# facebookresearch/omni3d

Measured on AMD Instinct MI355X. Metric: images/sec train DLA34_FPN b=4/GPU, higher is better.
Workload: dtype f32; 1 GPU; cubercnn_DLA34_FPN train step, batch 4/GPU, synthetic Omni3D 512x512 (8 GT/img), fwd+10 losses+bwd+allreduce+divergence guard+SGD, random-init weights; global_batch=4, image=512x512, parallelism=dp1 (flat-bucket RCCL all-reduce)

## Files before the change

include/omni3d_hip.h:

```cpp
#ifndef OMNI3D_HIP_H
#define OMNI3D_HIP_H

#ifdef __cplusplus
extern "C" {
#endif


int omni_iou_box3d(const float* boxes1, int N, const float* boxes2, int M, const int* valid1, float* vol,
                   float* iou, int* overflow, void* stream);

int omni_iou_box3d_pairs(const float* boxes1, const float* boxes2, const int* idx1, const int* idx2,
                         long long npairs, const int* valid1, float* vol, float* iou, int* overflow,
                         void* stream);

int omni_iou_box3d_pairs_algo(const float* boxes1, const float* boxes2, const int* idx1, const int* idx2,
                              long long npairs, const int* valid1, float* vol, float* iou, int* overflow,
                              int lanes_per_pair, void* stream);

int omni_box3d_validity(const float* boxes, int N, float eps_coplanar, float eps_nonzero, int* valid,
                        int* counts, void* stream);


int omni_conv2d_fwd(const float* x, const float* w, const float* bias, float* out, int N, int H, int W, int C,
                    int K, int R, int S, int stride, int pad, int ldx, int ldo, int relu, void* stream);
// ... 160 lines not shown
int omni_rpn_collect(const float* boxes, const float* top_v, const int* top_i, int B, int N, int P, float* prop,
                     int* count, void* stream);

int omni_roi_sample(const float* prop_boxes, const int* prop_count, int B, int pmax, const float* gt,
                    const int* gt_cls, const int* gt_off, const float* ign, const int* ign_off, const float* expo,
                    float iou_thr, float ignore_thresh, float eps, int num_classes, int batch_per_image,
                    int nfg_max, int append_gt, float* out_boxes, int* out_cls, int* out_gt, float* out_iou,
                    int* out_counts, void* stream);
int omni_rpn_match_draw(const float* anchors, int A, const float* gt, const int* gt_off, int B, int G, float thr_lo,
                        float thr_hi, int l0, int l1, int l2, int allow_low_quality, const float* expo, long long* draw_state,
                        int* ticket, float eps, float* matched_val, int* matched_idx, signed char* match_label, int* gt_best_bits,
                        int* gt_best_idx, float* key_pos, float* key_neg, void* stream);
int omni_roi_sample_draw(const float* prop_boxes, const int* prop_count, int B, int pmax, const float* gt, const int* gt_cls,
                         const int* gt_off, const float* ign, const int* ign_off, const float* expo, long long* draw_state, int* ticket,
                         float iou_thr, float ignore_thresh, float eps, int num_classes, int batch_per_image, int nfg_max,
                         int append_gt, float* out_boxes, int* out_cls, int* out_gt, float* out_iou, int* out_counts, int* out_row,
                         int first, float* first_boxes, int* first_cls, int* first_row, void* stream);


int omni_roi_levels(const float* rois, int R, int min_level, int max_level, float canonical_size,
                    int canonical_level, int* levels, void* stream);

int omni_roi_align_fwd(const void* const* level_ptrs, const int* level_hw, const float* level_scale, int nlev,
                       const float* rois, const int* batch_idx, const int* levels, int R, int P, int C,
                       float* out, void* stream);
int omni_roi_align_fwd_mode(const void* const* level_ptrs, const int* level_hw, const float* level_scale, int nlev,
                            const float* rois, const int* batch_idx, const int* levels, int R, int P, int C, int aligned, float* out,
                            void* stream);
int omni_roi_align_bwd_mode(const void* const* dlevel_ptrs, const int* level_hw, const float* level_scale, int nlev,
                            const float* rois, const int* batch_idx, const int* levels, int R, int P, int C, int aligned,
                            const float* dout, void* stream);
int omni_roi_pool_fwd(const void* const* level_ptrs, const int* level_hw, const float* level_scale, int nlev, const float* rois,
                      const int* batch_idx, const int* levels, int R, int P, int C, float* out, int* argmax, void* stream);
int omni_roi_pool_bwd(const void* const* dlevel_ptrs, const int* level_hw, const float* level_scale, int nlev, const int* batch_idx,
                      const int* levels, int R, int P, int C, const float* dout, const int* argmax, void* stream);
int omni_roi_align_fwd2(const void* const* level_ptrs, const int* level_hw, const float* level_scale, int nlev,
                        const float* rois, const int* batch_idx, const int* levels, int R, int P, int C, float* out,
                        float* out2, int per_image, int first, void* stream);
int omni_roi_align_bwd(const void* const* dlevel_ptrs, const int* level_hw, const float* level_scale, int nlev,
                       const float* rois, const int* batch_idx, const int* levels, int R, int P, int C,
                       const float* dout, void* stream);
int omni_roi_align_bwd2(const void* const* dlevel_ptrs, const int* level_hw, const float* level_scale, int nlev,
                        const float* rois, const int* batch_idx, const int* levels, int R, int P, int C,
                        const float* dout, const float* dout2, int per_image, int first, void* stream);
int omni_roi_align_bwd_det(const void* const* dlevel_ptrs, const int* level_hw, const float* level_scale, int nlev, int B,
                           const float* rois, const int* batch_idx, const int* levels, int R, int P, int C, const float* dout,
                           const float* dout2, int per_image, int first, float* ws, long long ws_floats, int* ctr, int n_ctr,
                           long long* plan, void* stream);


int omni_box_loss_fwd(const float* pred, int ldp, int R, int K, const int* cls, const float* prop, const float* gt,
                      const int* gt_row, float wx, float wy, float ww, float wh, double* sums, void* stream);
int omni_box_loss_bwd(const float* pred, int ldp, int R, int K, const int* cls, const float* prop, const float* gt,
                      const int* gt_row, float wx, float wy, float ww, float wh, const double* sums,
                      const float* g_cls, const float* g_reg, float* dpred, void* stream);

int omni_box_decode_gt_class(const float* pred, int ldp, int R, int K, const int* cls, const float* prop, float wx, float wy,
                             float ww, float wh, float scale_clamp, float* out, void* stream);

int omni_cube_loss_fwd(const float* head, int ldh, int F, int K, int mode, int bins, const float* zscales, const float* zstats,
                       const float* boxes, const int* cls, const int* img,
                       const float* Ks, const float* v2r, const float* priors, const float* gt3d,
                       const float* gtpose, const int* gt_row, float w_dims, float w_pose, float w_xy, float w_z, float w_joint,
                       float* vals, float* jac, float* red, void* stream);
int omni_cube_loss_bwd(const float* vals, const float* jac, const float* red, const float* gk, const int* cls,
                       const float* boxes, int F, int K, int mode, int bins, const float* zscales, int ldh, float* dhead,
                       void* stream);
int omni_cube_decode(const float* head, int ldh, int F, int K, int mode, int bins, const float* zscales, const float* zstats,
                     const float* boxes, const int* cls, const int* img,
                     const float* Ks, const float* v2r, const float* ratio, const float* priors, float* cube3d,
                     float* pose, float* verts, void* stream);
int omni_cuboid_corners(const float* box3d, const float* R, int n, float* verts, void* stream);

int omni_conv2d_fwd_stats(const float* x, const float* w, float* out, int N, int H, int W, int C, int K, int R, int S,
                          int stride, int pad, int ldx, int ldo, float* stats, int stats_rows, int* nblk_out, void* stream);
int omni_wino_out_stats(const float* M, float* y, int N, int H, int W, int K, int tile, float* stats, int stats_rows,
                        int* nblk_out, void* stream);
int omni_wino_out_bn_bwd_stats(const float* M, float* y, int N, int H, int W, int K, int tile, const float* bn_x,
                               const float* mean_rstd, const float* scale_shift, float* stats, int stats_rows, int* nblk_out,
                               void* stream);
int omni_bn_bwd_partials(const float* x, const float* dy, const float* y, const float* gamma, const float* mean_rstd,
                         const float* partial, int nblk, float* dx, float* dres, float* dgamma, float* dbeta, float* coef,
                         int P, int C, int relu, int accumulate_param_grads, void* stream);
int omni_stem_conv_fwd_stats(const float* x, const float* w, float* out, int N, int H, int W, int C, int K, int R, int ldx,
                             int ldo, float* stats, int stats_rows, int* nblk_out, void* stream);
int omni_bn_fwd_partials(const float* x, const float* partial, int nblk, const float* gamma, const float* beta,
                         const float* residual, float* y, float* running_mean, float* running_var, float* mean_rstd,
                         float* scale_shift, int P, int C, float eps, float momentum, int relu, void* stream);

int omni_gemm_engine(const float* A, const float* B, float* C, const float* bias, int form, int batch, int M, int N, int K,
                     int lda, int ldb, int ldc, long long stride_a, long long stride_b, long long stride_c, int splits,
                     int relu, int accumulate, int tile, int workgroups, void* stream);
int omni_gemm_engine_det(const float* A, const float* B, float* C, const float* bias, int form, int batch, int M, int N, int K,
                         int lda, int ldb, int ldc, long long stride_a, long long stride_b, long long stride_c, int splits,
                         int relu, int accumulate, int tile, int workgroups, float* ws, long long ws_floats, int* ctr, int n_ctr,
                         long long* plan, void* stream);

int omni_transpose2d(const float* src, float* dst, int rows, int cols, void* stream);

int omni_det_scores(const float* pred, int ld, const float* rois, const int* count, const int* image_hw, int B, int P, int K,
                    float wx, float wy, float ww, float wh, float score_thresh, float* scores, float* probs, float* boxes,
                    void* stream);
int omni_det_nms_boxes(const float* boxes, const float* vals, const int* idx, int B, int PK, int K, int cap, float* nms_boxes,
                       int* valid, void* stream);
int omni_det_compact(const int* keep, const int* valid, const float* vals, const int* idx, const float* boxes, int B, int PK,
                     int K, int cap, int topk, float* out_box, float* out_score, int* out_cls, int* out_roi, int* out_count,
                     void* stream);

int omni_resize_bilinear_u8(const unsigned char* src, unsigned char* dst, unsigned char* tmp, int planes, int H, int W,
                            int HO, int WO, const int* bounds_h, const int* kk_h, int ksize_h, const int* bounds_v,
                            const int* kk_v, int ksize_v, int flip, void* stream);


int omni_sgd_step(float* param, const float* grad, float* momentum_buf, long long n, float lr, float momentum,
                  float dampening, float weight_decay, int nesterov, int first_step, float grad_scale,
                  const float* skip_flag, void* stream);
int omni_adam_step(float* param, const float* grad, float* exp_avg, float* exp_avg_sq, float* max_exp_avg_sq, long long n, float lr,
                   float beta1, float beta2, float eps, float weight_decay, int decoupled, const float* step, float grad_scale,
                   const float* skip_flag, void* stream);
int omni_adam_tick(float* step, const float* skip_flag, void* stream);
int omni_clip_norm_partials(const float* grad, const long long* tiles, int ntiles, float norm_type, double* partial, void* stream);
int omni_clip_norm_coef(const double* partial, const long long* ptab, int nparams, float norm_type, float max_norm, float grad_scale,
                        float* norm, float* coef, void* stream);
int omni_sgd_step_clipped(float* param, const float* grad, float* momentum_buf, const long long* tiles, int t0, int t1, int clip_mode,
                          const float* coef, float clip_value, float lr, float momentum, float dampening, float weight_decay,
                          int nesterov, int first_step, float grad_scale, const float* skip_flag, void* stream);
int omni_adam_step_clipped(float* param, const float* grad, float* exp_avg, float* exp_avg_sq, float* max_exp_avg_sq,
                           const long long* tiles, int t0, int t1, int clip_mode, const float* coef, float clip_value, float lr,
                           float beta1, float beta2, float eps, float weight_decay, int decoupled, const float* step,
                           float grad_scale, const float* skip_flag, void* stream);
int omni_guard_pre(float* vec, int n, void* stream);
int omni_guard_post(float* vec, int n, int world, float stabilize, float half_period, float tolerance, float gamma, float* state,
                    float* skip, float* out, void* stream);
int omni_scale_vec(const void* src, int src_f64, int stride, const double* coef, const void* denom, double denom_min, int n, float* out,
                   void* stream);
int omni_sum_vectors(const void* const* vecs, const int* lens, int nvec, int nfirst, float* out, void* stream);
int omni_guard_gather(const void* const* scalars, int n, float* vec, void* stream);
int omni_bump_counters(const void* const* counters, int n, long long delta, void* stream);
int omni_zero(void* p, long long nbytes, void* stream);
int omni_nonfinite_any(const float* grad, long long n, float* flag, void* stream);

int omni_relu_bwd(const float* dy, const float* y, float* dz, long long n, void* stream);
int omni_bias_grad(const float* dy, int P, int C, float* db, double* ws, int accumulate, void* stream);

int omni_maxpool3s2_fwd(const float* x, float* y, int N, int H, int W, int C, void* stream);
int omni_maxpool3s2_bwd(const float* x, const float* dy, float* dx, int N, int H, int W, int C, void* stream);

int omni_wino_in(const float* x, float* V, int N, int H, int W, int C, int tile, void* stream);
int omni_wino_out(const float* M, const float* bias, float* y, int N, int H, int W, int K, int relu, int tile, void* stream);
int omni_wino_dy(const float* dy, float* dM, int N, int H, int W, int K, int tile, void* stream);
int omni_wino_weights_multi(const void* const* g, const void* const* U, const void* const* U_flip, const int* K, const int* C,
                            const int* tile, int n, void* stream);
int omni_wino_dy_in(const float* dy, float* dM, float* Vd, int N, int H, int W, int K, int tile, void* stream);
int omni_wino_weights(const float* g, float* U , float* U_flip , int K, int C, int tile, void* stream);
int omni_wino_dweights(const float* dU, float* dg, int K, int C, int accumulate, int tile, void* stream);
int omni_wino_dweights_multi(const void* const* dU, const void* const* dg, const int* K, const int* C, const int* tile, int n,
                             void* stream);
int omni_gemm_batched_fwd(const float* x, const float* w, float* out, int batch, int M, int C, int K, void* stream);
int omni_gemm_batched_fwd_algo(const float* x, const float* w, float* out, int batch, int M, int C, int K, int algo,
                               int workgroups, void* stream);
int omni_gemm_batched_wgrad(const float* x, const float* dy, float* dw, int batch, int M, int C, int K, void* stream);
int omni_gemm_batched_wgrad_algo(const float* x, const float* dy, float* dw, int batch, int M, int C, int K, int algo,
                                 void* stream);
int omni_gemm_batched_wgrad_det(const float* x, const float* dy, float* dw, int batch, int M, int C, int K, int algo, float* ws,
                                long long ws_floats, int* ctr, int n_ctr, long long* plan, void* stream);
int omni_gemm_batched_wgrad_multi(const void* const* x, const void* const* dy, const void* const* dw, const int* batch, const int* M,
// ... 35 lines not shown
```

omni3d_amd/csrc/bn_pool.hip:

```cpp
#include <device_rt.h>

namespace {

__device__ __forceinline__ float4 ld4(const float* p) { return *reinterpret_cast<const float4*>(p); }
__device__ __forceinline__ void st4(float* p, float4 v) { *reinterpret_cast<float4*>(p) = v; }
__device__ __forceinline__ float4 f4(float a) { return make_float4(a, a, a, a); }
__device__ __forceinline__ float4 relu4(float4 a) { return make_float4(fmaxf(a.x, 0.f), fmaxf(a.y, 0.f), fmaxf(a.z, 0.f), fmaxf(a.w, 0.f)); }
__device__ __forceinline__ float4 mask4(float4 g, float4 y) {
    return make_float4(y.x > 0.f ? g.x : 0.f, y.y > 0.f ? g.y : 0.f, y.z > 0.f ? g.z : 0.f, y.w > 0.f ? g.w : 0.f);
}

template <int MODE>
__device__ __forceinline__ void bn_reduce_tile(const float* __restrict__ x, const float* __restrict__ dy,
                                               const float* __restrict__ y, const float* __restrict__ mean_rstd,
                                               int P, int C, int relu, double* __restrict__ acc, int cbase, int C4,
                                               float4* __restrict__ s0, float4* __restrict__ s1, long lddy) {
    const int rows = 256 / C4;
    const int t = threadIdx.x;
    const int col = cbase + t % C4, row = t / C4;
    const bool active = row < rows;
    float4 a0 = f4(0.f), a1 = f4(0.f);
    float4 mu = f4(0.f), rs = f4(0.f), sc = f4(0.f), sh = f4(0.f);
    if (MODE == 1 && active) { mu = ld4(mean_rstd + 4 * col); rs = ld4(mean_rstd + C + 4 * col); }
    if (MODE == 1 && active && relu == 2) { sc = ld4(y + 4 * col); sh = ld4(y + C + 4 * col); }
    if (active) {
        const long step = (long)gridDim.x * rows;
        long p = (long)blockIdx.x * rows + row;
        for (; p + 3 * step < P; p += 4 * step) {
            float4 xv[4], g[4];
#pragma unroll
            for (int u = 0; u < 4; ++u) xv[u] = ld4(x + (p + u * step) * C + 4 * col);
            if (MODE == 0) {
#pragma unroll
                for (int u = 0; u < 4; ++u) { a0 = a0 + xv[u]; a1 = a1 + xv[u] * xv[u]; }
            } else {
#pragma unroll
                for (int u = 0; u < 4; ++u) g[u] = ld4(dy + (p + u * step) * lddy + 4 * col);
                if (relu == 1) {
#pragma unroll
                    for (int u = 0; u < 4; ++u) g[u] = mask4(g[u], ld4(y + (p + u * step) * C + 4 * col));
                } else if (relu == 2) {
#pragma unroll
                    for (int u = 0; u < 4; ++u) g[u] = mask4(g[u], xv[u] * sc + sh);
                }
#pragma unroll
                for (int u = 0; u < 4; ++u) { a0 = a0 + g[u]; a1 = a1 + g[u] * ((xv[u] - mu) * rs); }
            }
        }
        for (; p < P; p += step) {
            const long off = p * C + 4 * col;
            const float4 xv = ld4(x + off);
            if (MODE == 0) {
                a0 = a0 + xv;
                a1 = a1 + xv * xv;
            } else {
                float4 g = ld4(dy + p * lddy + 4 * col);
                if (relu == 1) g = mask4(g, ld4(y + off));
                else if (relu == 2) g = mask4(g, xv * sc + sh);
                a0 = a0 + g;
                a1 = a1 + g * ((xv - mu) * rs);
            }
        }
    }
    s0[t] = a0;
    s1[t] = a1;
    __syncthreads();
    if (t < C4) {
        float4 r0 = s0[t], r1 = s1[t];
        for (int r = 1; r < rows; ++r) { r0 = r0 + s0[r * C4 + t]; r1 = r1 + s1[r * C4 + t]; }
        float* a = reinterpret_cast<float*>(acc) + (long)blockIdx.x * 2 * C;
        st4(a + 4 * (cbase + t), r0);
        st4(a + C + 4 * (cbase + t), r1);
    }
}
template <int MODE>
__device__ __forceinline__ void bn_reduce_body(const float* __restrict__ x, const float* __restrict__ dy,
                                               const float* __restrict__ y, const float* __restrict__ mean_rstd,
                                               int P, int C, int relu, double* __restrict__ acc, long lddy = 0) {
    __shared__ float4 s0[256], s1[256];
    if (lddy == 0) lddy = C;
    const int C4 = C >> 2;
    for (int cbase = 0; cbase < C4; cbase += 256) {
        const int width = C4 - cbase < 256 ? C4 - cbase : 256;
// ... 397 lines not shown
    if (partial == nullptr) return;
    s0[t] = a0;
    s1[t] = a1;
    __syncthreads();
    for (int half = 32; half >= 1; half >>= 1) {
        if (prow < half) { s0[t] = s0[t] + s0[t + half * GQ]; s1[t] = s1[t] + s1[t + half * GQ]; }
        __syncthreads();
    }
    if (prow == 0 && active) {
        st4(partial + (long)pc * 2 * C + coff, s0[t]);
        st4(partial + (long)pc * 2 * C + C + coff, s1[t]);
    }
}

__global__ void __launch_bounds__(256) bn_frozen_bwd_fin_kernel(const float* __restrict__ partial, int nblk, int C, float* __restrict__ dgamma,
                                                                float* __restrict__ dbeta, int accumulate) {
    double db, dg;
    colsum_fin(partial, nblk, C, blockIdx.x * FIN_C, db, dg);
    const int c = blockIdx.x * FIN_C + threadIdx.x;
    if (threadIdx.x >= FIN_C || c >= C) return;
    dbeta[c] = accumulate ? dbeta[c] + (float)db : (float)db;
    dgamma[c] = accumulate ? dgamma[c] + (float)dg : (float)dg;
}

#ifndef OMNI_HIPEMU
__global__ void __launch_bounds__(256) bias_grad_atomic_kernel(const float* __restrict__ dy, int P, int C, float* __restrict__ db) {
    __shared__ float4 s0[256];
    const int C4 = C >> 2, rows = 256 / C4, t = threadIdx.x, col = t % C4, row = t / C4;
    float4 a = f4(0.f);
    if (row < rows) {
        const long step = (long)gridDim.x * rows;
        long p = (long)blockIdx.x * rows + row;
        for (; p + 3 * step < P; p += 4 * step) {
            float4 v[4];
#pragma unroll
            for (int u = 0; u < 4; ++u) v[u] = ld4(dy + (p + u * step) * C + 4 * col);
            a = a + ((v[0] + v[1]) + (v[2] + v[3]));
        }
        for (; p < P; p += step) a = a + ld4(dy + p * C + 4 * col);
    }
    s0[t] = a;
    __syncthreads();
    if (t < C4) {
        float4 r = s0[t];
        for (int k = 1; k < rows; ++k) r = r + s0[k * C4 + t];
        atomicAdd(db + 4 * t + 0, r.x); atomicAdd(db + 4 * t + 1, r.y); atomicAdd(db + 4 * t + 2, r.z); atomicAdd(db + 4 * t + 3, r.w);
    }
}
#endif

__global__ void __launch_bounds__(256) maxpool2_fwd_kernel(const float* __restrict__ x, float* __restrict__ y, int N,
                                                           int H, int W, int C) {
    const int C4 = C >> 2, OH = H >> 1, OW = W >> 1;
    const long total = (long)N * OH * OW * C4;
    for (long i = (long)blockIdx.x * blockDim.x + threadIdx.x; i < total; i += (long)gridDim.x * blockDim.x) {
        const int col = (int)(i % C4);
        long q = i / C4;
        const int ow = (int)(q % OW); q /= OW;
        const int oh = (int)(q % OH);
        const int n = (int)(q / OH);
        const float* b = x + (((long)n * H + 2 * oh) * W + 2 * ow) * C + 4 * col;
        const float4 v00 = ld4(b), v01 = ld4(b + C), v10 = ld4(b + (long)W * C), v11 = ld4(b + (long)W * C + C);
        float4 m;
        m.x = fmaxf(fmaxf(v00.x, v01.x), fmaxf(v10.x, v11.x));
        m.y = fmaxf(fmaxf(v00.y, v01.y), fmaxf(v10.y, v11.y));
        m.z = fmaxf(fmaxf(v00.z, v01.z), fmaxf(v10.z, v11.z));
        m.w = fmaxf(fmaxf(v00.w, v01.w), fmaxf(v10.w, v11.w));
        st4(y + 4 * i, m);
    }
}

__device__ __forceinline__ void route(float v00, float v01, float v10, float v11, float g, float& d00, float& d01,
                                      float& d10, float& d11) {
    int k = 0;
    float m = v00;
    if (v01 > m) { m = v01; k = 1; }
    if (v10 > m) { m = v10; k = 2; }
    if (v11 > m) { m = v11; k = 3; }
    d00 = k == 0 ? g : 0.f; d01 = k == 1 ? g : 0.f; d10 = k == 2 ? g : 0.f; d11 = k == 3 ? g : 0.f;
}

__global__ void __launch_bounds__(256) maxpool2_bwd_kernel(const float* __restrict__ x, const float* __restrict__ dy,
                                                           float* __restrict__ dx, int N, int H, int W, int C,
                                                           const float* __restrict__ carry, long ldc, long lddy) {
    const int C4 = C >> 2, OH = H >> 1, OW = W >> 1;
    const long total = (long)N * OH * OW * C4;
    for (long i = (long)blockIdx.x * blockDim.x + threadIdx.x; i < total; i += (long)gridDim.x * blockDim.x) {
        const int col = (int)(i % C4);
        long q = i / C4;
        const int ow = (int)(q % OW); q /= OW;
        const int oh = (int)(q % OH);
        const int n = (int)(q / OH);
        const long o = (((long)n * H + 2 * oh) * W + 2 * ow) * C + 4 * col;
        const float4 v00 = ld4(x + o), v01 = ld4(x + o + C), v10 = ld4(x + o + (long)W * C), v11 = ld4(x + o + (long)W * C + C);
        const float4 g = ld4(dy + (i / C4) * lddy + 4 * col);
        float4 d00, d01, d10, d11;
        route(v00.x, v01.x, v10.x, v11.x, g.x, d00.x, d01.x, d10.x, d11.x);
        route(v00.y, v01.y, v10.y, v11.y, g.y, d00.y, d01.y, d10.y, d11.y);
        route(v00.z, v01.z, v10.z, v11.z, g.z, d00.z, d01.z, d10.z, d11.z);
        route(v00.w, v01.w, v10.w, v11.w, g.w, d00.w, d01.w, d10.w, d11.w);
        if (carry != nullptr) {
            const long pc = (((long)n * H + 2 * oh) * W + 2 * ow) * ldc + 4 * col;
            d00 = d00 + ld4(carry + pc); d01 = d01 + ld4(carry + pc + ldc);
            d10 = d10 + ld4(carry + pc + (long)W * ldc); d11 = d11 + ld4(carry + pc + (long)W * ldc + ldc);
        }
        st4(dx + o, d00); st4(dx + o + C, d01); st4(dx + o + (long)W * C, d10); st4(dx + o + (long)W * C + C, d11);
    }
}

template <int DIR>
__global__ void __launch_bounds__(256) avgpool2_kernel(const float* __restrict__ src, float* __restrict__ dst, int N, int H, int W,
                                                       int C) {
    const int C4 = C >> 2, OH = H >> 1, OW = W >> 1;
    const long total = (long)N * OH * OW * C4;
    for (long i = (long)blockIdx.x * blockDim.x + threadIdx.x; i < total; i += (long)gridDim.x * blockDim.x) {
        const int col = (int)(i % C4);
        long q = i / C4;
        const int ow = (int)(q % OW); q /= OW;
        const int oh = (int)(q % OH);
        const int n = (int)(q / OH);
        const long o = (((long)n * H + 2 * oh) * W + 2 * ow) * C + 4 * col;
        if (DIR == 0) {
            const float4 a = ld4(src + o), b = ld4(src + o + C), c = ld4(src + o + (long)W * C), d = ld4(src + o + (long)W * C + C);
            float4 m;
            m.x = (a.x + b.x + c.x + d.x) * 0.25f; m.y = (a.y + b.y + c.y + d.y) * 0.25f;
            m.z = (a.z + b.z + c.z + d.z) * 0.25f; m.w = (a.w + b.w + c.w + d.w) * 0.25f;
            st4(dst + 4 * i, m);
        } else {
            float4 g = ld4(src + 4 * i);
            g.x *= 0.25f; g.y *= 0.25f; g.z *= 0.25f; g.w *= 0.25f;
            st4(dst + o, g); st4(dst + o + C, g); st4(dst + o + (long)W * C, g); st4(dst + o + (long)W * C + C, g);
        }
    }
}

__global__ void __launch_bounds__(256) subsample2_bwd_carry_kernel(const float* __restrict__ dy, const float* __restrict__ carry, long ldc,
                                                                   float* __restrict__ dx, int N, int H, int W, int C) {
    const int C4 = C >> 2, OH = (H - 1) / 2 + 1, OW = (W - 1) / 2 + 1;
    const long total = (long)N * H * W * C4;
    for (long i = (long)blockIdx.x * blockDim.x + threadIdx.x; i < total; i += (long)gridDim.x * blockDim.x) {
        const int col = (int)(i % C4);
        long q = i / C4;
        const long pix = q;
        const int w = (int)(q % W); q /= W;
        const int h = (int)(q % H);
        const int n = (int)(q / H);
        float4 v = ld4(carry + pix * ldc + 4 * col);
        if (!((h | w) & 1)) v = v + ld4(dy + ((((long)n * OH + (h >> 1)) * OW + (w >> 1)) * C4 + col) * 4);
        st4(dx + 4 * i, v);
    }
}

template <int DIR>
__global__ void __launch_bounds__(256) subsample2_kernel(const float* __restrict__ src, float* __restrict__ dst, int N,
                                                         int H, int W, int C) {
    const int C4 = C >> 2, OH = (H - 1) / 2 + 1, OW = (W - 1) / 2 + 1;
    const long total = (long)N * OH * OW * C4;
    for (long i = (long)blockIdx.x * blockDim.x + threadIdx.x; i < total; i += (long)gridDim.x * blockDim.x) {
        const int col = (int)(i % C4);
        long q = i / C4;
        const int ow = (int)(q % OW); q /= OW;
        const int oh = (int)(q % OH);
        const int n = (int)(q / OH);
        const long big = (((long)n * H + 2 * oh) * W + 2 * ow) * C + 4 * col;
        if (DIR == 0) st4(dst + 4 * i, ld4(src + big));
        else st4(dst + big, ld4(src + 4 * i));
    }
}

__global__ void __launch_bounds__(256) upsample2_add_kernel(const float* __restrict__ lat, const float* __restrict__ top,
                                                            float* __restrict__ out, int N, int H, int W, int C) {
    const int C4 = C >> 2, TH = H >> 1, TW = W >> 1;
    const long total = (long)N * H * W * C4;
    for (long i = (long)blockIdx.x * blockDim.x + threadIdx.x; i < total; i += (long)gridDim.x * blockDim.x) {
        const int col = (int)(i % C4);
        long q = i / C4;
        const int w = (int)(q % W); q /= W;
        const int h = (int)(q % H);
        const int n = (int)(q / H);
        const float4 t = ld4(top + (((long)n * TH + (h >> 1)) * TW + (w >> 1)) * C + 4 * col);
        st4(out + 4 * i, ld4(lat + 4 * i) + t);
    }
}

__global__ void __launch_bounds__(256) upsample2_bwd_kernel(const float* __restrict__ dout, float* __restrict__ dtop,
                                                            int N, int H, int W, int C, const float* __restrict__ carry, long ldc) {
    const int C4 = C >> 2, TH = H >> 1, TW = W >> 1;
    const long total = (long)N * TH * TW * C4;
    for (long i = (long)blockIdx.x * blockDim.x + threadIdx.x; i < total; i += (long)gridDim.x * blockDim.x) {
        const int col = (int)(i % C4);
// ... 62 lines not shown

}

extern "C" {

static inline void fin_geometry(int P, int C, int& CG, int& PC, int& chunk, int& grid) {
    CG = (C + GC - 1) / GC;
    long pc = 512 / CG;
    const long maxpc = ((long)P + 63) / 64;
    if (pc > maxpc) pc = maxpc;
    if (pc < 1) pc = 1;
    chunk = (int)((((long)P + pc - 1) / pc + 63) / 64 * 64);
    PC = (int)(((long)P + chunk - 1) / chunk);
    grid = (CG * PC + 7) / 8 * 8;
}
static inline bool fin_fusable(int C, int nblk, int fuse_rows) { return fuse_rows > 0 && nblk <= fuse_rows && (C % GC) == 0; }
static const int BN_FUSE_ROWS_DEFAULT = 512;

int omni_bn_fwd_algo(const float* x, const float* partial, int nblk, const float* gamma, const float* beta, const float* residual,
                     float* y, long long ldy, float* running_mean, float* running_var, float* mean_rstd, float* scale_shift, double* ws,
                     int P, int C, float eps, float momentum, int relu, int fuse_rows, void* stream) {
    if (P <= 0 || C <= 0 || (C & 3) || C > 4096 || (partial != nullptr && nblk <= 0) || (partial == nullptr && ws == nullptr))
        return OMNI_ERR_ARG;
    if (ldy == 0) ldy = C;
    if (ldy < C || (ldy & 3) || (((unsigned long long)y) & 15)) return OMNI_ERR_ARG;
    hipStream_t st = (hipStream_t)stream;
    if (partial == nullptr) {
        nblk = red_grid(P, C);
        float* mine = reinterpret_cast<float*>(ws + 2 * C);
        hipLaunchKernelGGL(HIP_KERNEL_NAME(bn_reduce_kernel<0>), dim3(nblk), dim3(256), 0, st, x, (const float*)nullptr,
                           (const float*)nullptr, (const float*)nullptr, P, C, 0, reinterpret_cast<double*>(mine), 0L);
        partial = mine;
    }
    if (fin_fusable(C, nblk, fuse_rows)) {
        int CG, PC, chunk, grid;
        fin_geometry(P, C, CG, PC, chunk, grid);
        hipLaunchKernelGGL(bn_fin_apply_kernel, dim3(grid), dim3(256), 0, st, x, partial, nblk, P, C, eps, momentum, gamma, beta, residual,
                           y, (long)ldy, mean_rstd, scale_shift, running_mean, running_var, relu, CG, PC, chunk);
        return omni_launch_status();
    }
    hipLaunchKernelGGL(bn_finalize_fwd_kernel, dim3((C + FIN_C - 1) / FIN_C), dim3(256), 0, st, partial, nblk, P, C, eps, momentum, gamma,
                       beta, mean_rstd, scale_shift, running_mean, running_var);
    const long total4 = (long)P * (C >> 2);
    hipLaunchKernelGGL(bn_apply_kernel, dim3(ew_grid(total4)), dim3(256), 0, st, x, (const float*)scale_shift, residual, y, total4, C, relu,
                       (long)ldy);
    return omni_launch_status();
}

int omni_bn_fwd(const float* x, const float* gamma, const float* beta, const float* residual, float* y,
                float* running_mean, float* running_var, float* mean_rstd, float* scale_shift, double* ws, int P, int C,
                float eps, float momentum, int relu, void* stream) {
    return omni_bn_fwd_algo(x, nullptr, 0, gamma, beta, residual, y, C, running_mean, running_var, mean_rstd, scale_shift, ws, P, C, eps,
                            momentum, relu, BN_FUSE_ROWS_DEFAULT, stream);
}

int omni_bn_fwd_partials(const float* x, const float* partial, int nblk, const float* gamma, const float* beta, const float* residual,
                         float* y, float* running_mean, float* running_var, float* mean_rstd, float* scale_shift, int P, int C,
                         float eps, float momentum, int relu, void* stream) {
    if (partial == nullptr) return OMNI_ERR_ARG;
    return omni_bn_fwd_algo(x, partial, nblk, gamma, beta, residual, y, C, running_mean, running_var, mean_rstd, scale_shift, nullptr, P, C,
                            eps, momentum, relu, BN_FUSE_ROWS_DEFAULT, stream);
}

int omni_bn_apply(const float* x, const float* scale_shift, const float* residual, float* y, int P, int C, int relu,
                  void* stream) {
    if (P <= 0 || C <= 0 || (C & 3)) return OMNI_ERR_ARG;
    const long total4 = (long)P * (C >> 2);
    hipLaunchKernelGGL(bn_apply_kernel, dim3(ew_grid(total4)), dim3(256), 0, (hipStream_t)stream, x, scale_shift, residual,
                       y, total4, C, relu, 0L);
    return omni_launch_status();
}

static int bad_carry(const float* carry, long long ldc, int C) {
    return carry != nullptr && (ldc < C || (ldc & 3) || (((unsigned long long)carry) & 15));
}

int omni_bn_bwd_algo(const float* x, const float* dy, long long lddy, const float* y, const float* gamma, const float* mean_rstd,
                     const float* partial, int nblk, float* dx, float* dres, const float* res_carry, long long ldc, float* dgamma,
                     float* dbeta, double* ws, float* coef, int P, int C, int relu, int accumulate_param_grads, int fuse_rows,
                     void* stream) {
    if (P <= 0 || C <= 0 || (C & 3) || C > 4096 || relu < 0 || relu > 2 || (relu && y == nullptr)) return OMNI_ERR_ARG;
    if (lddy == 0) lddy = C;
    if (bad_carry(res_carry, ldc, C) || (res_carry != nullptr && dres == nullptr) || bad_carry(dy, lddy, C)) return OMNI_ERR_ARG;
    if ((partial != nullptr && (nblk <= 0 || res_carry != nullptr || lddy != C)) || (partial == nullptr && ws == nullptr)) return OMNI_ERR_ARG;
    hipStream_t st = (hipStream_t)stream;
    if (partial == nullptr) {
        nblk = red_grid(P, C);
        float* mine = reinterpret_cast<float*>(ws + 2 * C);
        hipLaunchKernelGGL(HIP_KERNEL_NAME(bn_reduce_kernel<1>), dim3(nblk), dim3(256), 0, st, x, dy, y, mean_rstd, P, C, relu,
                           reinterpret_cast<double*>(mine), (long)lddy);
        partial = mine;
    }
    if (fin_fusable(C, nblk, fuse_rows)) {
        int CG, PC, chunk, grid;
        fin_geometry(P, C, CG, PC, chunk, grid);
        hipLaunchKernelGGL(bn_fin_bwd_apply_kernel, dim3(grid), dim3(256), 0, st, x, dy, (long)lddy, y, mean_rstd, gamma, partial, nblk, P, C,
                           dgamma, dbeta, accumulate_param_grads, dx, dres, res_carry, (long)ldc, relu, CG, PC, chunk);
        return omni_launch_status();
    }
    if (coef == nullptr) return OMNI_ERR_ARG;
    hipLaunchKernelGGL(bn_finalize_bwd_kernel, dim3((C + FIN_C - 1) / FIN_C), dim3(256), 0, st, partial, nblk, P, C, gamma, mean_rstd,
                       dgamma, dbeta, coef, accumulate_param_grads);
    const long total4 = (long)P * (C >> 2);
    hipLaunchKernelGGL(bn_bwd_apply_kernel, dim3(ew_grid(total4)), dim3(256), 0, st, x, dy, y, mean_rstd,
                       (const float*)coef, dx, dres, total4, C, relu, res_carry, (long)ldc, (long)lddy);
    return omni_launch_status();
}

int omni_bn_bwd_carry(const float* x, const float* dy, long long lddy, const float* y, const float* gamma, const float* mean_rstd, float* dx,
                      float* dres, const float* res_carry, long long ldc, float* dgamma, float* dbeta, double* ws, float* coef, int P,
                      int C, int relu, int accumulate_param_grads, void* stream) {
    return omni_bn_bwd_algo(x, dy, lddy, y, gamma, mean_rstd, nullptr, 0, dx, dres, res_carry, ldc, dgamma, dbeta, ws, coef, P, C, relu,
                            accumulate_param_grads, BN_FUSE_ROWS_DEFAULT, stream);
}

int omni_bn_bwd(const float* x, const float* dy, const float* y, const float* gamma, const float* mean_rstd, float* dx,
                float* dres, float* dgamma, float* dbeta, double* ws, float* coef, int P, int C, int relu,
                int accumulate_param_grads, void* stream) {
    return omni_bn_bwd_carry(x, dy, C, y, gamma, mean_rstd, dx, dres, nullptr, 0, dgamma, dbeta, ws, coef, P, C, relu,
                             accumulate_param_grads, stream);
}

int omni_bn_bwd_partials(const float* x, const float* dy, const float* y, const float* gamma, const float* mean_rstd,
                         const float* partial, int nblk, float* dx, float* dres, float* dgamma, float* dbeta, float* coef, int P,
                         int C, int relu, int accumulate_param_grads, void* stream) {
    if (partial == nullptr) return OMNI_ERR_ARG;
    return omni_bn_bwd_algo(x, dy, C, y, gamma, mean_rstd, partial, nblk, dx, dres, nullptr, 0, dgamma, dbeta, nullptr, coef, P, C, relu,
                            accumulate_param_grads, BN_FUSE_ROWS_DEFAULT, stream);
}

int omni_bn_frozen_fwd(const float* x, const float* gamma, const float* beta, const float* running_mean, const float* running_var,
                       float eps, const float* residual, float* y, int P, int C, int relu, void* stream) {
    if (P <= 0 || C <= 0 || (C & 3) || C > 4096 || !gamma || !beta || !running_mean || !running_var) return OMNI_ERR_ARG;
    int CG, PC, chunk, grid;
    fin_geometry(P, C, CG, PC, chunk, grid);
    hipLaunchKernelGGL(bn_frozen_fwd_kernel, dim3(grid), dim3(256), 0, (hipStream_t)stream, x, gamma, beta, running_mean, running_var, eps,
                       residual, y, P, C, relu, CG, PC, chunk);
    return omni_launch_status();
}

int omni_bn_frozen_bwd(const float* x, const float* dy, long long lddy, const float* y, const float* gamma, const float* beta,
                       const float* running_mean, const float* running_var, float eps, float* dx, float* dres, const float* res_carry,
                       long long ldc, float* dgamma, float* dbeta, float* ws, long long ws_floats, int P, int C, int relu,
                       int accumulate_param_grads, void* stream) {
    if (P <= 0 || C <= 0 || (C & 3) || C > 4096 || relu < 0 || relu > 2 || (relu == 1 && y == nullptr)) return OMNI_ERR_ARG;
    if (!gamma || !beta || !running_mean || !running_var || (dgamma == nullptr) != (dbeta == nullptr)) return OMNI_ERR_ARG;
    if (lddy == 0) lddy = C;
    if (bad_carry(res_carry, ldc, C) || (res_carry != nullptr && dres == nullptr) || bad_carry(dy, lddy, C)) return OMNI_ERR_ARG;
    int CG, PC, chunk, grid;
    fin_geometry(P, C, CG, PC, chunk, grid);
    const bool params = dgamma != nullptr;
    if (params && (ws == nullptr || ws_floats < 2LL * C * PC)) return OMNI_ERR_ARG;
    hipStream_t st = (hipStream_t)stream;
    hipLaunchKernelGGL(bn_frozen_bwd_kernel, dim3(grid), dim3(256), 0, st, x, dy, (long)lddy, y, gamma, beta, running_mean, running_var, eps,
                       dx, dres, res_carry, (long)ldc, params ? ws : nullptr, P, C, relu, CG, PC, chunk);
    if (params)
        hipLaunchKernelGGL(bn_frozen_bwd_fin_kernel, dim3((C + FIN_C - 1) / FIN_C), dim3(256), 0, st, (const float*)ws, PC, C, dgamma, dbeta,
                           accumulate_param_grads);
    return omni_launch_status();
}

int omni_maxpool2_fwd(const float* x, float* y, int N, int H, int W, int C, void* stream) {
    if ((C & 3) || H < 2 || W < 2) return OMNI_ERR_ARG;
    const long total = (long)N * (H / 2) * (W / 2) * (C / 4);
    if (total == 0) return OMNI_OK;
    hipLaunchKernelGGL(maxpool2_fwd_kernel, dim3(ew_grid(total)), dim3(256), 0, (hipStream_t)stream, x, y, N, H, W, C);
    return omni_launch_status();
}

int omni_maxpool2_bwd_carry(const float* x, const float* dy, long long lddy, const float* carry, long long ldc, float* dx, int N, int H,
                            int W, int C, void* stream) {
    if ((C & 3) || H < 2 || W < 2 || bad_carry(carry, ldc, C) || (carry != nullptr && ((H & 1) || (W & 1))) || bad_carry(dy, lddy, C))
        return OMNI_ERR_ARG;
    const long total = (long)N * (H / 2) * (W / 2) * (C / 4);
    if (total == 0) return OMNI_OK;
    if ((H & 1) || (W & 1)) omni_memset_async(dx, 0, sizeof(float) * (size_t)N * H * W * C, (hipStream_t)stream);
    hipLaunchKernelGGL(maxpool2_bwd_kernel, dim3(ew_grid(total)), dim3(256), 0, (hipStream_t)stream, x, dy, dx, N, H, W, C, carry, (long)ldc,
                       (long)lddy);
    return omni_launch_status();
}

int omni_maxpool2_bwd(const float* x, const float* dy, float* dx, int N, int H, int W, int C, void* stream) {
    return omni_maxpool2_bwd_carry(x, dy, C, nullptr, 0, dx, N, H, W, C, stream);
}

int omni_avgpool2_fwd(const float* x, float* y, int N, int H, int W, int C, void* stream) {
    if ((C & 3) || H < 2 || W < 2) return OMNI_ERR_ARG;
    const long total = (long)N * (H / 2) * (W / 2) * (C / 4);
    if (total == 0) return OMNI_OK;
    hipLaunchKernelGGL(HIP_KERNEL_NAME(avgpool2_kernel<0>), dim3(ew_grid(total)), dim3(256), 0, (hipStream_t)stream, x, y, N, H, W, C);
    return omni_launch_status();
}

int omni_avgpool2_bwd(const float* dy, float* dx, int N, int H, int W, int C, void* stream) {
    if ((C & 3) || H < 2 || W < 2) return OMNI_ERR_ARG;
    const long total = (long)N * (H / 2) * (W / 2) * (C / 4);
    if (total == 0) return OMNI_OK;
    if ((H & 1) || (W & 1)) omni_memset_async(dx, 0, sizeof(float) * (size_t)N * H * W * C, (hipStream_t)stream);
    hipLaunchKernelGGL(HIP_KERNEL_NAME(avgpool2_kernel<1>), dim3(ew_grid(total)), dim3(256), 0, (hipStream_t)stream, dy, dx, N, H, W, C);
    return omni_launch_status();
}

int omni_subsample2_fwd(const float* x, float* y, int N, int H, int W, int C, void* stream) {
    if (C & 3) return OMNI_ERR_ARG;
    const long total = (long)N * ((H - 1) / 2 + 1) * ((W - 1) / 2 + 1) * (C / 4);
    if (total == 0) return OMNI_OK;
    hipLaunchKernelGGL(HIP_KERNEL_NAME(subsample2_kernel<0>), dim3(ew_grid(total)), dim3(256), 0, (hipStream_t)stream, x,
                       y, N, H, W, C);
    return omni_launch_status();
}

int omni_subsample2_bwd(const float* dy, float* dx, int N, int H, int W, int C, void* stream) {
    if (C & 3) return OMNI_ERR_ARG;
    const long total = (long)N * ((H - 1) / 2 + 1) * ((W - 1) / 2 + 1) * (C / 4);
    omni_memset_async(dx, 0, sizeof(float) * (size_t)N * H * W * C, (hipStream_t)stream);
    if (total == 0) return OMNI_OK;
    hipLaunchKernelGGL(HIP_KERNEL_NAME(subsample2_kernel<1>), dim3(ew_grid(total)), dim3(256), 0, (hipStream_t)stream, dy,
                       dx, N, H, W, C);
    return omni_launch_status();
}

int omni_subsample2_bwd_carry(const float* dy, const float* carry, long long ldc, float* dx, int N, int H, int W, int C, void* stream) {
    if ((C & 3) || carry == nullptr || bad_carry(carry, ldc, C)) return OMNI_ERR_ARG;
    const long total = (long)N * H * W * (C / 4);
    if (total == 0) return OMNI_OK;
    hipLaunchKernelGGL(subsample2_bwd_carry_kernel, dim3(ew_grid(total)), dim3(256), 0, (hipStream_t)stream, dy, carry, (long)ldc, dx, N, H,
                       W, C);
    return omni_launch_status();
}

int omni_upsample2_add(const float* lat, const float* top, float* out, int N, int H, int W, int C, void* stream) {
    if ((C & 3) || (H & 1) || (W & 1)) return OMNI_ERR_ARG;
    const long total = (long)N * H * W * (C / 4);
    if (total == 0) return OMNI_OK;
    hipLaunchKernelGGL(upsample2_add_kernel, dim3(ew_grid(total)), dim3(256), 0, (hipStream_t)stream, lat, top, out, N, H,
                       W, C);
    return omni_launch_status();
}

int omni_upsample2_bwd_carry(const float* dout, const float* carry, long long ldc, float* dtop, int N, int H, int W, int C, void* stream) {
    if ((C & 3) || (H & 1) || (W & 1) || bad_carry(carry, ldc, C)) return OMNI_ERR_ARG;
    const long total = (long)N * (H / 2) * (W / 2) * (C / 4);
    if (total == 0) return OMNI_OK;
    hipLaunchKernelGGL(upsample2_bwd_kernel, dim3(ew_grid(total)), dim3(256), 0, (hipStream_t)stream, dout, dtop, N, H, W, C, carry, (long)ldc);
    return omni_launch_status();
}

int omni_upsample2_bwd(const float* dout, float* dtop, int N, int H, int W, int C, void* stream) {
    return omni_upsample2_bwd_carry(dout, nullptr, 0, dtop, N, H, W, C, stream);
}

int omni_preprocess_masked(const unsigned char* img, const int* image_hw, float* out, int N, int H, int W, int PH, int PW, float m0,
                           float m1, float m2, float s0, float s1, float s2, void* stream) {
    if (PH < H || PW < W) return OMNI_ERR_ARG;
    const long total = (long)N * PH * PW;
    if (total == 0) return OMNI_OK;
    hipLaunchKernelGGL(HIP_KERNEL_NAME(preprocess_kernel<false>), dim3(ew_grid(total)), dim3(256), 0, (hipStream_t)stream, img, ImgPtrs{}, out, N, H,
                       W, PH, PW, m0, m1, m2, s0, s1, s2, image_hw);
    return omni_launch_status();
}

int omni_preprocess_multi(const void* const* imgs, const int* image_hw, float* out, int N, int H, int W, int PH, int PW, float m0,
// ... 46 lines not shown
```

omni3d_amd/csrc/stem_conv.hip:

```cpp
#include <device_rt.h>

namespace {

__device__ __forceinline__ float4 ld4(const float* p) { return *reinterpret_cast<const float4*>(p); }

template <int C, int R, bool ROT = false>
__global__ void __launch_bounds__(256) stem_conv_fwd_kernel(const float* __restrict__ x, const float* __restrict__ w,
                                                            float* __restrict__ out, int N, int H, int W, int ldx, int ldo,
                                                            float* __restrict__ stats, int cw) {
    static_assert(!ROT || C == 16, "the rotated form is the 16 -> 16 layer's data gradient");
    constexpr int TH = 4, TW = 64, PAD = R / 2;
    constexpr int HR = TH + R - 1, HC = TW + R - 1 + (C == 4 ? 1 : 0);
    constexpr int PP = (C == 16) ? 20 : 4;
    constexpr int SP = (C == 16) ? R : 8;
    constexpr int KD = R * SP * C;
    constexpr int KP = KD + ((KD / 4) % 2 == 0 ? 4 : 8);
    __shared__ __attribute__((aligned(16))) float s_in[HR * HC * PP];
    __shared__ __attribute__((aligned(16))) float s_w[16 * KP];
    const int tid = threadIdx.x, lane = tid & 63, wave = tid >> 6;
    const int tiles_x = (W + TW - 1) / TW, tiles_y = (H + TH - 1) / TH;
    int t = blockIdx.x;
    const int tx = t % tiles_x; t /= tiles_x;
    const int ty = t % tiles_y;
    const int n = t / tiles_y;
    const int oy0 = ty * TH, ox0 = tx * TW;

    constexpr int C4 = C / 4;
    constexpr int NI = (HR * HC * C4 + 255) / 256, NW = (16 * R * SP * C4 + 255) / 256;
    float4 vi[NI], vw[NW];
#pragma unroll
    for (int u = 0; u < NI; ++u) {
        const int i = tid + 256 * u;
        const int c4 = i % C4, col = (i / C4) % HC, row = i / (C4 * HC);
        const int iy = oy0 - PAD + row, ix = ox0 - PAD + col;
        vi[u] = make_float4(0.f, 0.f, 0.f, 0.f);
        if (i < HR * HC * C4 && (unsigned)iy < (unsigned)H && (unsigned)ix < (unsigned)W)
            vi[u] = ld4(x + (((long)n * H + iy) * W + ix) * ldx + 4 * c4);
    }
#pragma unroll
    for (int u = 0; u < NW; ++u) {
        const int i = tid + 256 * u;
        const int c4 = i % C4, s = (i / C4) % SP, r = (i / (C4 * SP)) % R, k = i / (C4 * SP * R);
        vw[u] = make_float4(0.f, 0.f, 0.f, 0.f);
        if (i < 16 * R * SP * C4 && s < R) {
            if (C != 4 || cw == C) {
                vw[u] = ld4(w + (((long)k * R + r) * R + s) * C + 4 * c4);
            } else {
                const float* q = w + (((long)k * R + r) * R + s) * cw;
                vw[u].x = q[0];
                vw[u].y = cw > 1 ? q[1] : 0.f;
                vw[u].z = cw > 2 ? q[2] : 0.f;
            }
        }
    }
#pragma unroll
    for (int u = 0; u < NI; ++u) {
        const int i = tid + 256 * u;
        const int c4 = i % C4, col = (i / C4) % HC, row = i / (C4 * HC);
        if (i < HR * HC * C4) *reinterpret_cast<float4*>(s_in + (row * HC + col) * PP + 4 * c4) = vi[u];
    }
#pragma unroll
    for (int u = 0; u < NW; ++u) {
        const int i = tid + 256 * u;
        const int c4 = i % C4, s = (i / C4) % SP, r = (i / (C4 * SP)) % R, k = i / (C4 * SP * R);
        if (i < 16 * R * SP * C4) {
            if (ROT) {
                float* q = s_w + (4 * c4) * KP + ((R - 1 - r) * SP + (R - 1 - s)) * C + k;
                q[0] = vw[u].x; q[KP] = vw[u].y; q[2 * KP] = vw[u].z; q[3 * KP] = vw[u].w;
            } else {
                *reinterpret_cast<float4*>(s_w + k * KP + (r * SP + s) * C + 4 * c4) = vw[u];
            }
        }
    }
    __syncthreads();

    const int px = lane & 15, g = lane >> 4;
    f32x4 acc[4];
#pragma unroll
    for (int b = 0; b < 4; ++b) acc[b] = (f32x4){0.f, 0.f, 0.f, 0.f};
    if (C == 16) {
#pragma unroll 1
        for (int r = 0; r < R; ++r)
#pragma unroll
            for (int s = 0; s < R; ++s) {
                const float4 bw = *reinterpret_cast<const float4*>(s_w + px * KP + (r * SP + s) * C + 4 * g);
#pragma unroll
                for (int b = 0; b < 4; ++b) {
                    const float4 a = *reinterpret_cast<const float4*>(s_in + ((wave + r) * HC + 16 * b + px + s) * PP + 4 * g);
                    acc[b] = mfma_16x16x4(a.x, bw.x, acc[b]);
                    acc[b] = mfma_16x16x4(a.y, bw.y, acc[b]);
                    acc[b] = mfma_16x16x4(a.z, bw.z, acc[b]);
                    acc[b] = mfma_16x16x4(a.w, bw.w, acc[b]);
                }
            }
    } else {
#pragma unroll 1
        for (int r = 0; r < R; ++r)
#pragma unroll
            for (int sg = 0; sg < SP / 4; ++sg) {
                const float4 bw = *reinterpret_cast<const float4*>(s_w + px * KP + (r * SP + 4 * sg + g) * C);
#pragma unroll
                for (int b = 0; b < 4; ++b) {
                    const float4 a = *reinterpret_cast<const float4*>(s_in + ((wave + r) * HC + 16 * b + px + 4 * sg + g) * PP);
                    acc[b] = mfma_16x16x4(a.x, bw.x, acc[b]);
                    acc[b] = mfma_16x16x4(a.y, bw.y, acc[b]);
                    acc[b] = mfma_16x16x4(a.z, bw.z, acc[b]);
                    acc[b] = mfma_16x16x4(a.w, bw.w, acc[b]);
                }
            }
    }
    const int oy = oy0 + wave;
    float sv = 0.f, sq = 0.f;
    if (oy < H) {
#pragma unroll
        for (int b = 0; b < 4; ++b)
#pragma unroll
            for (int i = 0; i < 4; ++i) {
                const int ox = ox0 + 16 * b + 4 * g + i;
                if (ox < W) {
                    out[(((long)n * H + oy) * W + ox) * ldo + px] = acc[b][i];
                    sv += acc[b][i];
                    sq += acc[b][i] * acc[b][i];
                }
            }
    }
    if (stats != nullptr) {
        sv += __shfl_xor(sv, 16, 64); sq += __shfl_xor(sq, 16, 64);
        sv += __shfl_xor(sv, 32, 64); sq += __shfl_xor(sq, 32, 64);
        __syncthreads();
        if (lane < 16) { s_in[wave * 32 + lane] = sv; s_in[wave * 32 + 16 + lane] = sq; }
        __syncthreads();
        if (tid < 32) stats[(long)blockIdx.x * 32 + tid] = s_in[tid] + s_in[32 + tid] + s_in[64 + tid] + s_in[96 + tid];
    }
}


template <int C, int K>
__global__ void __launch_bounds__(256) stem_dgrad_s2_kernel(const float* __restrict__ dy, const float* __restrict__ w,
                                                            float* __restrict__ dx, int N, int H, int W, int OH, int OW, int lddy,
                                                            int lddx) {
    static_assert(C == 16 && K % 16 == 0, "N = 16 dx channels per MFMA block; dy channels in chunks of 16");
    constexpr int TH = 8, TW = 64, HR = TH / 2 + 1, HC = TW / 2 + 1, PP = K + 4, KP = K + 4, K4 = K / 4, KH = K / 16;
    __shared__ __attribute__((aligned(16))) float s_dy[HR * HC * PP];
    __shared__ __attribute__((aligned(16))) float s_w[9 * C * KP];
    const int tid = threadIdx.x, lane = tid & 63, wave = tid >> 6;
    const int tiles_x = (W + TW - 1) / TW, tiles_y = (H + TH - 1) / TH;
    int t = blockIdx.x;
    const int tx = t % tiles_x; t /= tiles_x;
    const int ty = t % tiles_y;
    const int n = t / tiles_y;
    const int oy0 = ty * TH, ox0 = tx * TW;
    const int hy0 = oy0 / 2, hx0 = ox0 / 2;
    constexpr int NI = (HR * HC * K4 + 255) / 256, NW = (K * 9 * (C / 4) + 255) / 256;
    float4 vi[NI], vw[NW];
#pragma unroll
    for (int u = 0; u < NI; ++u) {
        const int i = tid + 256 * u;
        const int k4 = i % K4, col = (i / K4) % HC, row = i / (K4 * HC);
        const int oy = hy0 + row, ox = hx0 + col;
        vi[u] = make_float4(0.f, 0.f, 0.f, 0.f);
        if (i < HR * HC * K4 && oy < OH && ox < OW) vi[u] = ld4(dy + (((long)n * OH + oy) * OW + ox) * lddy + 4 * k4);
    }
#pragma unroll
    for (int u = 0; u < NW; ++u) {
        const int i = tid + 256 * u;
        vw[u] = make_float4(0.f, 0.f, 0.f, 0.f);
        if (i < K * 9 * (C / 4)) vw[u] = ld4(w + 4L * i);
    }
#pragma unroll
    for (int u = 0; u < NI; ++u) {
        const int i = tid + 256 * u;
        const int k4 = i % K4, col = (i / K4) % HC, row = i / (K4 * HC);
        if (i < HR * HC * K4) *reinterpret_cast<float4*>(s_dy + (row * HC + col) * PP + 4 * k4) = vi[u];
    }
#pragma unroll
    for (int u = 0; u < NW; ++u) {
        const int i = tid + 256 * u;
        if (i < K * 9 * (C / 4)) {
            const int c4 = i % (C / 4), tap = (i / (C / 4)) % 9, k = i / (9 * (C / 4));
            float* q = s_w + (tap * C + 4 * c4) * KP + k;
            q[0] = vw[u].x; q[KP] = vw[u].y; q[2 * KP] = vw[u].z; q[3 * KP] = vw[u].w;
        }
    }
    __syncthreads();

    const int px = lane & 15, g = lane >> 4;
#pragma unroll 1
    for (int half = 0; half < 2; ++half) {
        const int y = half == 0 ? wave : TH - 1 - wave;
        const int ih = oy0 + y;
        const int nr = 1 + (y & 1);
        f32x4 acc[2][2];
#pragma unroll
        for (int pw = 0; pw < 2; ++pw)
#pragma unroll
            for (int b = 0; b < 2; ++b) acc[pw][b] = (f32x4){0.f, 0.f, 0.f, 0.f};
#pragma unroll 1
        for (int jr = 0; jr < nr; ++jr) {
            const int r = (y & 1) ? 2 * jr : 1;
            const int lr = (y + 1 - r) >> 1;
#pragma unroll
            for (int pw = 0; pw < 2; ++pw)
#pragma unroll
                for (int js = 0; js <= pw; ++js) {
                    const int sx = pw ? 2 * js : 1, dc = pw ? 1 - js : 0;
#pragma unroll
                    for (int h2 = 0; h2 < KH; ++h2) {
                        const float4 bw = *reinterpret_cast<const float4*>(s_w + ((r * 3 + sx) * C + px) * KP + 16 * h2 + 4 * g);
#pragma unroll
                        for (int b = 0; b < 2; ++b) {
                            const float4 a = *reinterpret_cast<const float4*>(s_dy + (lr * HC + 16 * b + px + dc) * PP + 16 * h2 + 4 * g);
                            acc[pw][b] = mfma_16x16x4(a.x, bw.x, acc[pw][b]);
                            acc[pw][b] = mfma_16x16x4(a.y, bw.y, acc[pw][b]);
                            acc[pw][b] = mfma_16x16x4(a.z, bw.z, acc[pw][b]);
                            acc[pw][b] = mfma_16x16x4(a.w, bw.w, acc[pw][b]);
                        }
                    }
                }
        }
        if (ih < H) {
            float* orow = dx + ((long)n * H + ih) * W * lddx + px;
#pragma unroll
            for (int b = 0; b < 2; ++b)
#pragma unroll
                for (int i = 0; i < 4; ++i)
#pragma unroll
                    for (int pw = 0; pw < 2; ++pw) {
                        const int iw = ox0 + 2 * (16 * b + 4 * g + i) + pw;
                        if (iw < W) orow[(long)iw * lddx] = acc[pw][b][i];
                    }
        }
    }
}

template <int C, int R, int S, int K>
__global__ void __launch_bounds__(256) stem_conv_wgrad_kernel(const float* __restrict__ x, const float* __restrict__ dy,
                                                              float* __restrict__ dw, int N, int H, int W, int OH, int OW, int ldx,
                                                              int lddy, float* __restrict__ part) {
    constexpr int TH = 4, TW = (S == 1) ? 64 : 32, PAD = R / 2, KB = K / 16, K4 = K / 4;
    constexpr int HR = S * (TH - 1) + R, HC = S * (TW - 1) + R + (C == 4 ? 1 : 0);
    constexpr int NB = (C == 16) ? R * R : R * 2;
    constexpr int KD = R * R * C, E = K * KD;
    constexpr int IN_FLOATS = HR * HC * C, DY_FLOATS = TH * TW * K;
    static_assert(E <= IN_FLOATS + DY_FLOATS, "the filter gradient is summed over the waves in the tile buffers");
    static_assert(C == 16 || S == 1, "the 4-channel form walks 4 adjacent taps per block");
    __shared__ __attribute__((aligned(16))) float smem[IN_FLOATS + DY_FLOATS];
    float* s_in = smem;
    float* s_dy = smem + IN_FLOATS;
    const int tid = threadIdx.x, lane = tid & 63, wave = tid >> 6;
    const int col = lane & 15, g = lane >> 4;
    const int tiles_x = (OW + TW - 1) / TW, tiles_y = (OH + TH - 1) / TH;
    const int tiles = N * tiles_y * tiles_x;
    f32x4 acc[KB][NB];
#pragma unroll
    for (int kb = 0; kb < KB; ++kb)
#pragma unroll
        for (int b = 0; b < NB; ++b) acc[kb][b] = (f32x4){0.f, 0.f, 0.f, 0.f};
    constexpr int C4 = C / 4;
    for (int tile = blockIdx.x; tile < tiles; tile += gridDim.x) {
        int t = tile;
        const int tx = t % tiles_x; t /= tiles_x;
        const int ty = t % tiles_y;
        const int n = t / tiles_y;
        const int oy0 = ty * TH, ox0 = tx * TW;
        constexpr int NI = (HR * HC * C4 + 255) / 256, ND = (TH * TW * K4 + 255) / 256;
        float4 vi[NI], vd[ND];
#pragma unroll
        for (int u = 0; u < NI; ++u) {
            const int i = tid + 256 * u;
            const int c4 = i % C4, cc = (i / C4) % HC, row = i / (C4 * HC);
            const int iy = S * oy0 - PAD + row, ix = S * ox0 - PAD + cc;
            vi[u] = make_float4(0.f, 0.f, 0.f, 0.f);
            if (i < HR * HC * C4 && (unsigned)iy < (unsigned)H && (unsigned)ix < (unsigned)W)
                vi[u] = ld4(x + (((long)n * H + iy) * W + ix) * ldx + 4 * c4);
        }
#pragma unroll
        for (int u = 0; u < ND; ++u) {
            const int i = tid + 256 * u;
            const int k4 = i % K4, cc = (i / K4) % TW, row = i / (K4 * TW);
            const int oy = oy0 + row, ox = ox0 + cc;
            vd[u] = make_float4(0.f, 0.f, 0.f, 0.f);
            if (i < TH * TW * K4 && oy < OH && ox < OW) vd[u] = ld4(dy + (((long)n * OH + oy) * OW + ox) * lddy + 4 * k4);
        }
        __syncthreads();
#pragma unroll
        for (int u = 0; u < NI; ++u) {
            const int i = tid + 256 * u;
            const int c4 = i % C4, cc = (i / C4) % HC, row = i / (C4 * HC);
            if (i < HR * HC * C4) *reinterpret_cast<float4*>(s_in + (row * HC + cc) * C + 4 * c4) = vi[u];
        }
#pragma unroll
        for (int u = 0; u < ND; ++u) {
            const int i = tid + 256 * u;
            const int k4 = i % K4, cc = (i / K4) % TW, row = i / (K4 * TW);
            if (i < TH * TW * K4) *reinterpret_cast<float4*>(s_dy + (row * TW + cc) * K + 4 * k4) = vd[u];
        }
        __syncthreads();
#pragma unroll 1
        for (int p0 = 0; p0 < TW; p0 += 4) {
            float a[KB];
#pragma unroll
            for (int kb = 0; kb < KB; ++kb) a[kb] = s_dy[(wave * TW + p0 + g) * K + kb * 16 + col];
            if (C == 16) {
#pragma unroll
                for (int r = 0; r < R; ++r)
#pragma unroll
                    for (int sx = 0; sx < R; ++sx) {
                        const float b = s_in[((S * wave + r) * HC + S * (p0 + g) + sx) * C + col];
#pragma unroll
                        for (int kb = 0; kb < KB; ++kb) acc[kb][r * R + sx] = mfma_16x16x4(a[kb], b, acc[kb][r * R + sx]);
                    }
            } else {
#pragma unroll
                for (int r = 0; r < R; ++r)
#pragma unroll
                    for (int blk = 0; blk < 2; ++blk) {
                        const float b = s_in[((wave + r) * HC + p0 + g + 4 * blk) * C + col];
#pragma unroll
                        for (int kb = 0; kb < KB; ++kb) acc[kb][r * 2 + blk] = mfma_16x16x4(a[kb], b, acc[kb][r * 2 + blk]);
                    }
            }
        }
    }
    for (int w = 0; w < 4; ++w) {
        __syncthreads();
        if (wave == w) {
#pragma unroll
            for (int kb = 0; kb < KB; ++kb)
#pragma unroll
                for (int b = 0; b < NB; ++b) {
                    int off;
                    bool ok = true;
                    if (C == 16) {
                        off = b * C + col;
                    } else {
                        const int r = b >> 1, sx = 4 * (b & 1) + (col >> 2);
                        ok = sx < R;
                        off = (r * R + sx) * C + (col & 3);
                    }
                    if (!ok) continue;
#pragma unroll
                    for (int i = 0; i < 4; ++i) {
                        float* q = smem + (kb * 16 + 4 * g + i) * KD + off;
                        *q = (w == 0) ? acc[kb][b][i] : *q + acc[kb][b][i];
                    }
                }
        }
    }
    __syncthreads();
    if (part != nullptr) {
        float* row = part + (long)blockIdx.x * E;
        for (int e = tid; e < E; e += 256) row[e] = smem[e];
    } else {
        for (int e = tid; e < E; e += 256) atomicAdd(dw + e, smem[e]);
    }
}

__global__ void __launch_bounds__(256) stem_wgrad_finalize_kernel(const float* __restrict__ part, int rows, int E, float* __restrict__ dw,
                                                                  int accumulate, int C, int cw) {
    __shared__ double sm[256];
    const int t = threadIdx.x, el = t & 3, rg = t >> 2;
    const int e = (int)blockIdx.x * 4 + el;
    double a = 0.0;
    if (e < E) {
        int r = rg;
        for (; r + 192 < rows; r += 256) {
            const float v0 = part[(long)r * E + e], v1 = part[(long)(r + 64) * E + e], v2 = part[(long)(r + 128) * E + e],
                        v3 = part[(long)(r + 192) * E + e];
            a += (double)v0;
            a += (double)v1;
            a += (double)v2;
            a += (double)v3;
        }
        for (; r < rows; r += 64) a += (double)part[(long)r * E + e];
    }
    sm[t] = a;
    __syncthreads();
    for (int s = 128; s >= 4; s >>= 1) {
        if (t < s) sm[t] += sm[t + s];
        __syncthreads();
    }
    if (t < 4 && e < E) {
        const int c = e % C;
        if (c < cw) {
            float* d = dw + (long)(e / C) * cw + c;
            *d = accumulate ? *d + (float)sm[t] : (float)sm[t];
        }
    }
}

}

extern "C" {

static int stem_fwd_impl(const float* x, const float* w, float* out, int N, int H, int W, int C, int K, int R, int ldx, int ldo,
                         float* stats, int stats_rows, int* nblk_out, void* stream, bool rot = false, int cw = 0) {
    if (nblk_out) *nblk_out = 0;
    if (cw == 0) cw = C;
    if (N < 0 || H <= 0 || W <= 0 || K != 16 || ldx < C || ldo < K || (ldx & 3) || (rot && C != 16)) return OMNI_ERR_ARG;
    if (cw != C && (C != 4 || cw < 1 || cw > 4)) return OMNI_ERR_ARG;
    if (!((C == 4 && R == 7) || (C == 16 && R == 3))) return OMNI_ERR_ARG;
    if (N == 0) return OMNI_OK;
    const long tiles = (long)N * ((H + 3) / 4) * ((W + 63) / 64);
    float* sp = (stats != nullptr && tiles <= stats_rows) ? stats : nullptr;
    if (sp && nblk_out) *nblk_out = (int)tiles;
    if (C == 4)
        hipLaunchKernelGGL(HIP_KERNEL_NAME(stem_conv_fwd_kernel<4, 7>), dim3((unsigned)tiles), dim3(256), 0, (hipStream_t)stream, x, w,
                           out, N, H, W, ldx, ldo, sp, cw);
    else if (rot)
        hipLaunchKernelGGL(HIP_KERNEL_NAME(stem_conv_fwd_kernel<16, 3, true>), dim3((unsigned)tiles), dim3(256), 0, (hipStream_t)stream, x, w,
                           out, N, H, W, ldx, ldo, sp, cw);
    else
        hipLaunchKernelGGL(HIP_KERNEL_NAME(stem_conv_fwd_kernel<16, 3>), dim3((unsigned)tiles), dim3(256), 0, (hipStream_t)stream, x, w,
                           out, N, H, W, ldx, ldo, sp, cw);
    return omni_launch_status();
}

int omni_stem_conv_fwd(const float* x, const float* w, float* out, int N, int H, int W, int C, int K, int R, int ldx, int ldo,
                       void* stream) {
    return stem_fwd_impl(x, w, out, N, H, W, C, K, R, ldx, ldo, nullptr, 0, nullptr, stream);
}

int omni_stem_conv_dgrad(const float* dy, const float* w, float* dx, int N, int H, int W, int C, int K, int R, int lddy, int lddx,
                         void* stream) {
    if (C != 16 || K != 16 || R != 3) return OMNI_ERR_ARG;
    return stem_fwd_impl(dy, w, dx, N, H, W, K, C, R, lddy, lddx, nullptr, 0, nullptr, stream, true);
}

int omni_stem_conv_s2_dgrad(const float* dy, const float* w, float* dx, int N, int H, int W, int C, int K, int R, int lddy, int lddx,
                            void* stream) {
    if (N < 0 || H <= 0 || W <= 0 || C != 16 || K != 32 || R != 3 || lddy < K || lddx < C || (lddy & 3)) return OMNI_ERR_ARG;
    if (N == 0) return OMNI_OK;
    const int OH = (H - 1) / 2 + 1, OW = (W - 1) / 2 + 1;
    const long tiles = (long)N * ((H + 7) / 8) * ((W + 63) / 64);
    if (tiles > 0x7fffffff) return OMNI_ERR_ARG;
    hipLaunchKernelGGL(HIP_KERNEL_NAME(stem_dgrad_s2_kernel<16, 32>), dim3((unsigned)tiles), dim3(256), 0, (hipStream_t)stream, dy, w, dx, N,
                       H, W, OH, OW, lddy, lddx);
    return omni_launch_status();
}

int omni_stem_conv_fwd_stats(const float* x, const float* w, float* out, int N, int H, int W, int C, int K, int R, int ldx, int ldo,
                             float* stats, int stats_rows, int* nblk_out, void* stream) {
    return stem_fwd_impl(x, w, out, N, H, W, C, K, R, ldx, ldo, stats, stats_rows, nblk_out, stream);
}

static int stem_wgrad_impl(const float* x, const float* dy, float* dw, int N, int H, int W, int C, int K, int R, int stride, int ldx,
                           int lddy, int accumulate, float* ws, long long ws_floats, long long* plan, bool det, void* stream, int cw = 0) {
    if (cw == 0) cw = C;
    if (N < 0 || H <= 0 || W <= 0 || ldx < C || lddy < K || (ldx & 3) || (lddy & 3)) return OMNI_ERR_ARG;
    if (cw != C && (!det || C != 4 || cw < 1 || cw > 4)) return OMNI_ERR_ARG;
    const int form = (C == 4 && R == 7 && stride == 1 && K == 16) ? 0 : (C == 16 && R == 3 && stride == 1 && K == 16) ? 1
                   : (C == 16 && R == 3 && stride == 2 && K == 32 && !(H & 1) && !(W & 1)) ? 2 : -1;
    if (form < 0) return OMNI_ERR_ARG;
    hipStream_t st = (hipStream_t)stream;
    const int OH = H / stride, OW = W / stride, TW = stride == 1 ? 64 : 32;
    const long tiles = (long)N * ((OH + 3) / 4) * ((OW + TW - 1) / TW);
    const long per = (tiles + 767) / 768;
    const unsigned grid = (unsigned)(tiles <= 768 ? tiles : (tiles + per - 1) / per);
    const int E = K * R * R * C;
    if (plan != nullptr) { plan[0] = plan[1] = plan[2] = 0; plan[3] = (long long)grid * E; return OMNI_OK; }
    if (det && N > 0 && (ws == nullptr || ws_floats < (long long)grid * E)) return OMNI_ERR_ARG;
    if (!accumulate && (!det || N == 0)) omni_memset_async(dw, 0, sizeof(float) * (size_t)(E / C * cw), st);
    if (N == 0) return OMNI_OK;
    float* part = det ? ws : nullptr;
    if (form == 0)
        hipLaunchKernelGGL(HIP_KERNEL_NAME(stem_conv_wgrad_kernel<4, 7, 1, 16>), dim3(grid), dim3(256), 0, st, x, dy, dw, N, H, W, OH, OW, ldx, lddy, part);
    else if (form == 1)
        hipLaunchKernelGGL(HIP_KERNEL_NAME(stem_conv_wgrad_kernel<16, 3, 1, 16>), dim3(grid), dim3(256), 0, st, x, dy, dw, N, H, W, OH, OW, ldx, lddy, part);
    else
        hipLaunchKernelGGL(HIP_KERNEL_NAME(stem_conv_wgrad_kernel<16, 3, 2, 32>), dim3(grid), dim3(256), 0, st, x, dy, dw, N, H, W, OH, OW, ldx, lddy, part);
    if (det)
        hipLaunchKernelGGL(stem_wgrad_finalize_kernel, dim3((unsigned)((E + 3) / 4)), dim3(256), 0, st, (const float*)part, (int)grid, E, dw,
                           accumulate, C, cw);
    return omni_launch_status();
}

int omni_stem_conv_wgrad(const float* x, const float* dy, float* dw, int N, int H, int W, int C, int K, int R, int ldx, int lddy,
                         int accumulate, void* stream) {
    return stem_wgrad_impl(x, dy, dw, N, H, W, C, K, R, 1, ldx, lddy, accumulate, nullptr, 0, nullptr, false, stream);
}

int omni_stem_conv_wgrad_det(const float* x, const float* dy, float* dw, int N, int H, int W, int C, int K, int R, int ldx, int lddy,
                             int accumulate, float* ws, long long ws_floats, long long* plan, void* stream) {
    return stem_wgrad_impl(x, dy, dw, N, H, W, C, K, R, 1, ldx, lddy, accumulate, ws, ws_floats, plan, true, stream);
}

int omni_stem_conv_fwd_cw(const float* x, const float* w, int cw, float* out, int N, int H, int W, int C, int K, int R, int ldx, int ldo,
                          float* stats, int stats_rows, int* nblk_out, void* stream) {
    return stem_fwd_impl(x, w, out, N, H, W, C, K, R, ldx, ldo, stats, stats_rows, nblk_out, stream, false, cw);
}
int omni_stem_conv_wgrad_det_cw(const float* x, const float* dy, float* dw, int cw, int N, int H, int W, int C, int K, int R, int ldx,
                                int lddy, int accumulate, float* ws, long long ws_floats, long long* plan, void* stream) {
    return stem_wgrad_impl(x, dy, dw, N, H, W, C, K, R, 1, ldx, lddy, accumulate, ws, ws_floats, plan, true, stream, cw);
}

int omni_stem_conv_s2_wgrad(const float* x, const float* dy, float* dw, int N, int H, int W, int C, int K, int R, int ldx, int lddy,
                            int accumulate, int deterministic, float* ws, long long ws_floats, long long* plan, void* stream) {
    return stem_wgrad_impl(x, dy, dw, N, H, W, C, K, R, 2, ldx, lddy, accumulate, ws, ws_floats, deterministic ? plan : nullptr,
                           deterministic != 0, stream);
}

}
```

omni3d_amd/csrc/winograd.hip:

```cpp
#include <device_rt.h>

namespace {

__device__ __forceinline__ float4 ld4(const float* p) { return *reinterpret_cast<const float4*>(p); }
__device__ __forceinline__ void st4(float* p, float4 v) { *reinterpret_cast<float4*>(p) = v; }
__device__ __forceinline__ float4 z4() { return make_float4(0.f, 0.f, 0.f, 0.f); }

inline int ew_grid(long total) {
    long g = (total + 255) / 256;
    if (g > 4096) g = 4096;
    return (int)(g < 1 ? 1 : g);
}

__device__ __forceinline__ float4 wino_ld(const float* __restrict__ p, bool ok, bool aff, float4 sc, float4 sh, int relu) {
    if (!ok) return z4();
    float4 v = ld4(p);
    if (aff) {
        v = v * sc + sh;
        if (relu) v = make_float4(fmaxf(v.x, 0.f), fmaxf(v.y, 0.f), fmaxf(v.z, 0.f), fmaxf(v.w, 0.f));
    }
    return v;
}

__global__ void __launch_bounds__(256) wino_in_kernel(const float* __restrict__ x, float* __restrict__ V, int N, int H, int W,
                                                      int C, const float* __restrict__ affine, int relu, long plane_in) {
    const int C4 = C >> 2, TH = H >> 1, TW = W >> 1;
    const bool aff = affine != nullptr;
    const long T = (long)N * TH * TW, total = T * C4, plane = plane_in > 0 ? plane_in : T * C;
    for (long i = (long)blockIdx.x * blockDim.x + threadIdx.x; i < total; i += (long)gridDim.x * blockDim.x) {
        const int c4 = (int)(i % C4);
        const long t = i / C4;
        const int tx = (int)(t % TW);
        const int ty = (int)((t / TW) % TH);
        const int n = (int)(t / ((long)TW * TH));
        const float4 sc = aff ? ld4(affine + 4 * c4) : z4(), sh = aff ? ld4(affine + C + 4 * c4) : z4();
        float4 d[4][4];
#pragma unroll
        for (int r = 0; r < 4; ++r) {
            const int ih = 2 * ty - 1 + r;
#pragma unroll
            for (int s = 0; s < 4; ++s) {
                const int iw = 2 * tx - 1 + s;
                const bool ok = (unsigned)ih < (unsigned)H && (unsigned)iw < (unsigned)W;
                d[r][s] = wino_ld(x + (((long)n * H + ih) * W + iw) * C + 4 * c4, ok, aff, sc, sh, relu);
            }
        }
        float4 u[4][4];
#pragma unroll
        for (int s = 0; s < 4; ++s) {
            u[0][s] = d[0][s] - d[2][s];
            u[1][s] = d[1][s] + d[2][s];
            u[2][s] = d[2][s] - d[1][s];
            u[3][s] = d[1][s] - d[3][s];
        }
        float* o = V + t * C + 4 * c4;
#pragma unroll
        for (int r = 0; r < 4; ++r) {
            st4(o + (long)(4 * r + 0) * plane, u[r][0] - u[r][2]);
            st4(o + (long)(4 * r + 1) * plane, u[r][1] + u[r][2]);
            st4(o + (long)(4 * r + 2) * plane, u[r][2] - u[r][1]);
            st4(o + (long)(4 * r + 3) * plane, u[r][1] - u[r][3]);
        }
    }
}

__device__ __forceinline__ void block_channel_stats(float4 sv, float4 sq, int K, float* __restrict__ stats) {
    __shared__ float4 r0[256], r1[256];
    const int K4 = K >> 2, t = threadIdx.x;
    r0[t] = sv;
    r1[t] = sq;
    __syncthreads();
    if (t < K4) {
        float4 a = r0[t], b = r1[t];
        for (int q = t + K4; q < 256; q += K4) {
            a = make_float4(a.x + r0[q].x, a.y + r0[q].y, a.z + r0[q].z, a.w + r0[q].w);
            b = make_float4(b.x + r1[q].x, b.y + r1[q].y, b.z + r1[q].z, b.w + r1[q].w);
        }
        st4(stats + (long)blockIdx.x * 2 * K + 4 * t, a);
        st4(stats + (long)blockIdx.x * 2 * K + K + 4 * t, b);
    }
}
#define OMNI_ACC_STATS(v) do { sv = make_float4(sv.x + (v).x, sv.y + (v).y, sv.z + (v).z, sv.w + (v).w); \
                               sq = make_float4(sq.x + (v).x * (v).x, sq.y + (v).y * (v).y, sq.z + (v).z * (v).z, sq.w + (v).w * (v).w); } while (0)

__global__ void __launch_bounds__(256) wino_out_kernel(const float* __restrict__ M, const float* __restrict__ bias,
                                                       float* __restrict__ y, int N, int H, int W, int K, int relu,
                                                       float* __restrict__ stats, const float* __restrict__ carry, long ldc, long plane_in) {
    const int K4 = K >> 2, TH = H >> 1, TW = W >> 1;
    const long T = (long)N * TH * TW, total = T * K4, plane = plane_in > 0 ? plane_in : T * K;
    float4 sv = z4(), sq = z4();
    for (long i = (long)blockIdx.x * blockDim.x + threadIdx.x; i < total; i += (long)gridDim.x * blockDim.x) {
        const int k4 = (int)(i % K4);
        const long t = i / K4;
        const int tx = (int)(t % TW);
        const int ty = (int)((t / TW) % TH);
        const int n = (int)(t / ((long)TW * TH));
        const float* m = M + t * K + 4 * k4;
        float4 s[2][4];
#pragma unroll
        for (int c = 0; c < 4; ++c) {
            const float4 m0 = ld4(m + (long)(0 + c) * plane), m1 = ld4(m + (long)(4 + c) * plane);
            const float4 m2 = ld4(m + (long)(8 + c) * plane), m3 = ld4(m + (long)(12 + c) * plane);
            s[0][c] = m0 + m1 + m2;
            s[1][c] = m1 - m2 - m3;
        }
        const float4 b = bias != nullptr ? ld4(bias + 4 * k4) : z4();
#pragma unroll
        for (int r = 0; r < 2; ++r) {
            float4 y0 = s[r][0] + s[r][1] + s[r][2] + b;
            float4 y1 = s[r][1] - s[r][2] - s[r][3] + b;
            if (relu) {
                y0 = make_float4(fmaxf(y0.x, 0.f), fmaxf(y0.y, 0.f), fmaxf(y0.z, 0.f), fmaxf(y0.w, 0.f));
                y1 = make_float4(fmaxf(y1.x, 0.f), fmaxf(y1.y, 0.f), fmaxf(y1.z, 0.f), fmaxf(y1.w, 0.f));
            }
            const long pix = ((long)n * H + 2 * ty + r) * W + 2 * tx;
            if (carry != nullptr) {
                y0 = y0 + ld4(carry + pix * ldc + 4 * k4);
                y1 = y1 + ld4(carry + (pix + 1) * ldc + 4 * k4);
            }
            float* o = y + pix * K + 4 * k4;
            st4(o, y0);
            st4(o + K, y1);
            OMNI_ACC_STATS(y0);
            OMNI_ACC_STATS(y1);
        }
    }
    if (stats != nullptr) block_channel_stats(sv, sq, K, stats);
}

__global__ void __launch_bounds__(256) wino_dy_kernel(const float* __restrict__ dy, float* __restrict__ dM, int N, int H, int W,
                                                      int K) {
    const int K4 = K >> 2, TH = H >> 1, TW = W >> 1;
    const long T = (long)N * TH * TW, total = T * K4, plane = T * K;
    for (long i = (long)blockIdx.x * blockDim.x + threadIdx.x; i < total; i += (long)gridDim.x * blockDim.x) {
        const int k4 = (int)(i % K4);
        const long t = i / K4;
        const int tx = (int)(t % TW);
        const int ty = (int)((t / TW) % TH);
        const int n = (int)(t / ((long)TW * TH));
        const float* g = dy + (((long)n * H + 2 * ty) * W + 2 * tx) * K + 4 * k4;
        const float4 g00 = ld4(g), g01 = ld4(g + K), g10 = ld4(g + (long)W * K), g11 = ld4(g + (long)W * K + K);
        float4 u[4][2];
        u[0][0] = g00;        u[0][1] = g01;
        u[1][0] = g00 + g10;  u[1][1] = g01 + g11;
        u[2][0] = g00 - g10;  u[2][1] = g01 - g11;
        u[3][0] = z4() - g10; u[3][1] = z4() - g11;
        float* o = dM + t * K + 4 * k4;
#pragma unroll
        for (int r = 0; r < 4; ++r) {
            st4(o + (long)(4 * r + 0) * plane, u[r][0]);
            st4(o + (long)(4 * r + 1) * plane, u[r][0] + u[r][1]);
            st4(o + (long)(4 * r + 2) * plane, u[r][0] - u[r][1]);
            st4(o + (long)(4 * r + 3) * plane, z4() - u[r][1]);
        }
    }
}

__device__ __forceinline__ void wino_w_body32(const float* __restrict__ g, float* __restrict__ U, float* __restrict__ Uf, int K, int C,
                                              int bid, float* __restrict__ smem) {
    float (*s_t)[32][33] = reinterpret_cast<float (*)[32][33]>(smem);
    const long total = (long)K * C;
    const int tiles_c = (C + 31) / 32;
    const int k0 = (bid / tiles_c) * 32, c0 = (bid % tiles_c) * 32;
    const int kq = threadIdx.x >> 5, cc = threadIdx.x & 31;
// ... 136 lines not shown
}

__global__ void __launch_bounds__(256) wino_dw_kernel(const float* __restrict__ dU, float* __restrict__ dg, int K, int C,
                                                      int accumulate) {
#pragma clang fp contract(off)
    const long total = (long)K * C;
    for (long i = (long)blockIdx.x * blockDim.x + threadIdx.x; i < total; i += (long)gridDim.x * blockDim.x) {
        const int c = (int)(i % C), k = (int)(i / C);
        float v[3][3];
        wino_dw_elem(dU, total, i, v);
#pragma unroll
        for (int r = 0; r < 3; ++r) {
            float* o = dg + ((long)k * 9 + r * 3) * C + c;
            if (accumulate) { o[0] += v[r][0]; o[C] += v[r][1]; o[2 * (long)C] += v[r][2]; }
            else { o[0] = v[r][0]; o[C] = v[r][1]; o[2 * (long)C] = v[r][2]; }
        }
    }
}

template <typename V>
__device__ __forceinline__ void bt6(const V (&d)[6], V (&t)[6]) {
    t[0] = d[0] + (d[3] - d[1]) * 1.5f - d[2] * 2.f + d[4];
    t[1] = d[2] * 0.5f + d[3] * 2.5f - d[1] + d[4];
    t[2] = d[1] - d[2] * 2.5f + d[3] * 0.5f + d[4];
    t[3] = (d[3] - d[1]) * 2.f - d[2] + d[4];
    t[4] = (d[1] - d[3]) * 0.5f - d[2] + d[4];
    t[5] = d[1] + (d[4] - d[2]) * 1.5f - d[3] * 2.f + d[5];
}
template <typename V>
__device__ __forceinline__ void at6(const V (&m)[6], V (&y)[4]) {
    y[0] = m[0] + m[1] + m[2] + m[3] + m[4];
    y[1] = m[1] - m[2] + m[3] * 0.5f - m[4] * 2.f;
    y[2] = m[1] + m[2] + m[3] * 0.25f + m[4] * 4.f;
    y[3] = m[1] - m[2] + m[3] * 0.125f - m[4] * 8.f + m[5];
}
template <typename V>
__device__ __forceinline__ void a6(const V (&y)[4], V (&u)[6]) {
    u[0] = y[0];
    u[1] = y[0] + y[1] + y[2] + y[3];
    u[2] = y[0] - y[1] + y[2] - y[3];
    u[3] = y[0] + y[1] * 0.5f + y[2] * 0.25f + y[3] * 0.125f;
    u[4] = y[0] - y[1] * 2.f + y[2] * 4.f - y[3] * 8.f;
    u[5] = y[3];
}

__global__ void __launch_bounds__(256) wino4_in_kernel(const float* __restrict__ x, float* __restrict__ V, int N, int H, int W,
                                                       int C, const float* __restrict__ affine, int relu, long plane_in) {
    const int C4 = C >> 2, TH = H >> 2, TW = W >> 2;
    const bool aff = affine != nullptr;
    const long T = (long)N * TH * TW, total = T * C4, plane = plane_in > 0 ? plane_in : T * C;
    for (long i = (long)blockIdx.x * blockDim.x + threadIdx.x; i < total; i += (long)gridDim.x * blockDim.x) {
        const int c4 = (int)(i % C4);
        const long t = i / C4;
        const int tx = (int)(t % TW);
        const int ty = (int)((t / TW) % TH);
        const int n = (int)(t / ((long)TW * TH));
        const float4 sc = aff ? ld4(affine + 4 * c4) : z4(), sh = aff ? ld4(affine + C + 4 * c4) : z4();
        float4 u[6][6];
#pragma unroll
        for (int s = 0; s < 6; ++s) {
            const int iw = 4 * tx - 1 + s;
            float4 d[6], tcol[6];
#pragma unroll
            for (int r = 0; r < 6; ++r) {
                const int ih = 4 * ty - 1 + r;
                const bool ok = (unsigned)ih < (unsigned)H && (unsigned)iw < (unsigned)W;
                d[r] = wino_ld(x + (((long)n * H + ih) * W + iw) * C + 4 * c4, ok, aff, sc, sh, relu);
            }
            bt6(d, tcol);
#pragma unroll
            for (int r = 0; r < 6; ++r) u[r][s] = tcol[r];
        }
        float* o = V + t * C + 4 * c4;
#pragma unroll
        for (int r = 0; r < 6; ++r) {
            float4 v[6];
            bt6(u[r], v);
#pragma unroll
            for (int s = 0; s < 6; ++s) st4(o + (long)(6 * r + s) * plane, v[s]);
        }
    }
}

struct BnBwdStats {
    const float* x;
    const float* mean_rstd;
    const float* scale_shift;
};
__global__ void __launch_bounds__(256) wino4_out_kernel(const float* __restrict__ M, const float* __restrict__ bias,
                                                        float* __restrict__ y, int N, int H, int W, int K, int relu,
                                                        float* __restrict__ stats, BnBwdStats bnb,
                                                        const float* __restrict__ carry, long ldc, long plane_in) {
    const int K4 = K >> 2, TH = H >> 2, TW = W >> 2;
    const long T = (long)N * TH * TW, total = T * K4, plane = plane_in > 0 ? plane_in : T * K;
    float4 sv = z4(), sq = z4();
    float4 mu = z4(), rs = z4(), sc = z4(), sh = z4();
    if (bnb.x != nullptr) {
        const int kc = 4 * (int)(threadIdx.x % K4);
        mu = ld4(bnb.mean_rstd + kc); rs = ld4(bnb.mean_rstd + K + kc);
        if (bnb.scale_shift != nullptr) { sc = ld4(bnb.scale_shift + kc); sh = ld4(bnb.scale_shift + K + kc); }
    }
    for (long i = (long)blockIdx.x * blockDim.x + threadIdx.x; i < total; i += (long)gridDim.x * blockDim.x) {
        const int k4 = (int)(i % K4);
        const long t = i / K4;
        const int tx = (int)(t % TW);
        const int ty = (int)((t / TW) % TH);
        const int n = (int)(t / ((long)TW * TH));
        const float* m = M + t * K + 4 * k4;
        float4 s[4][6];
#pragma unroll
        for (int c = 0; c < 6; ++c) {
            float4 col[6], o4[4];
#pragma unroll
            for (int r = 0; r < 6; ++r) col[r] = ld4(m + (long)(6 * r + c) * plane);
            at6(col, o4);
#pragma unroll
            for (int r = 0; r < 4; ++r) s[r][c] = o4[r];
        }
        const float4 b = bias != nullptr ? ld4(bias + 4 * k4) : z4();
#pragma unroll
        for (int r = 0; r < 4; ++r) {
            float4 row[4];
            at6(s[r], row);
            const long pix = ((long)n * H + 4 * ty + r) * W + 4 * tx;
            const long off = pix * K + 4 * k4;
            float* o = y + off;
            if (carry != nullptr) {
                float4 cv[4];
#pragma unroll
                for (int c = 0; c < 4; ++c) cv[c] = ld4(carry + (pix + c) * ldc + 4 * k4);
#pragma unroll
                for (int c = 0; c < 4; ++c) st4(o + (long)c * K, row[c] + cv[c]);
            } else if (bnb.x != nullptr) {
                float4 xv[4];
#pragma unroll
                for (int c = 0; c < 4; ++c) xv[c] = ld4(bnb.x + off + (long)c * K);
#pragma unroll
                for (int c = 0; c < 4; ++c) {
                    const float4 v = row[c];
                    st4(o + (long)c * K, v);
                    float4 g = v;
                    if (bnb.scale_shift != nullptr) {
                        const float4 yv = xv[c] * sc + sh;
                        g = make_float4(yv.x > 0.f ? v.x : 0.f, yv.y > 0.f ? v.y : 0.f, yv.z > 0.f ? v.z : 0.f, yv.w > 0.f ? v.w : 0.f);
                    }
                    const float4 xh = (xv[c] - mu) * rs;
                    sv = sv + g;
                    sq = sq + g * xh;
                }
            } else {
#pragma unroll
                for (int c = 0; c < 4; ++c) {
                    float4 v = row[c] + b;
                    if (relu) v = make_float4(fmaxf(v.x, 0.f), fmaxf(v.y, 0.f), fmaxf(v.z, 0.f), fmaxf(v.w, 0.f));
                    st4(o + (long)c * K, v);
                    OMNI_ACC_STATS(v);
                }
            }
        }
    }
    if (stats != nullptr) block_channel_stats(sv, sq, K, stats);
}

__global__ void __launch_bounds__(256) wino4_dy_kernel(const float* __restrict__ dy, float* __restrict__ dM, int N, int H, int W,
                                                       int K) {
    const int K4 = K >> 2, TH = H >> 2, TW = W >> 2;
    const long T = (long)N * TH * TW, total = T * K4, plane = T * K;
    for (long i = (long)blockIdx.x * blockDim.x + threadIdx.x; i < total; i += (long)gridDim.x * blockDim.x) {
        const int k4 = (int)(i % K4);
        const long t = i / K4;
        const int tx = (int)(t % TW);
        const int ty = (int)((t / TW) % TH);
        const int n = (int)(t / ((long)TW * TH));
        const float* g = dy + (((long)n * H + 4 * ty) * W + 4 * tx) * K + 4 * k4;
        float4 u[6][4];
#pragma unroll
        for (int c = 0; c < 4; ++c) {
            float4 col[4], o6[6];
#pragma unroll
            for (int r = 0; r < 4; ++r) col[r] = ld4(g + ((long)r * W + c) * K);
            a6(col, o6);
#pragma unroll
            for (int r = 0; r < 6; ++r) u[r][c] = o6[r];
        }
        float* o = dM + t * K + 4 * k4;
#pragma unroll
        for (int r = 0; r < 6; ++r) {
            float4 row[6];
            a6(u[r], row);
#pragma unroll
            for (int c = 0; c < 6; ++c) st4(o + (long)(6 * r + c) * plane, row[c]);
        }
    }
}

__device__ __forceinline__ void g6(const float (&g)[3], float (&a)[6]) {
    a[0] = g[0];
    a[1] = (g[0] + g[1] + g[2]) * (1.f / 3.f);
    a[2] = (g[1] - g[0] - g[2]) * (1.f / 3.f);
    a[3] = -(g[0] * 4.f + g[1] * 2.f + g[2]) * (4.f / 15.f);
    a[4] = (g[0] - g[1] * 2.f + g[2] * 4.f) * (1.f / 15.f);
    a[5] = g[2];
}
__device__ __forceinline__ void gt6(const float (&u)[6], float (&e)[3]) {
#pragma clang fp contract(off)
    e[0] = u[0] + (u[1] - u[2]) * (1.f / 3.f) - u[3] * (16.f / 15.f) + u[4] * (1.f / 15.f);
    e[1] = (u[1] + u[2]) * (1.f / 3.f) - u[3] * (8.f / 15.f) - u[4] * (2.f / 15.f);
    e[2] = (u[1] - u[2]) * (1.f / 3.f) + (u[4] - u[3]) * (4.f / 15.f) + u[5];
}

__device__ __forceinline__ void wino4_w_body(const float* __restrict__ g, float* __restrict__ U, float* __restrict__ Uf, int K, int C,
                                             int bid, float (*s_t)[16][17]) {
    const long total = (long)K * C;
    const int tiles_c = (C + 15) / 16;
    const int k0 = (bid / tiles_c) * 16, c0 = (bid % tiles_c) * 16;
    const int kk = threadIdx.x >> 4, cc = threadIdx.x & 15;
    const int k = k0 + kk, c = c0 + cc;
    const bool ok = k < K && c < C;
    float w[3][3];
#pragma unroll
    for (int r = 0; r < 3; ++r)
#pragma unroll
        for (int s = 0; s < 3; ++s) w[r][s] = ok ? g[((long)k * 9 + r * 3 + s) * C + c] : 0.f;
#pragma unroll
    for (int flip = 0; flip < 2; ++flip) {
        float* dst = flip ? Uf : U;
        if (dst == nullptr) continue;
        float a[6][3];
#pragma unroll
        for (int s = 0; s < 3; ++s) {
            float col[3], o6[6];
// ... 480 lines not shown
```

omni3d_amd/cubercnn/solver/graphed.py:

```python
import os

import torch

from ...functional import sum_vectors, total_loss


_units = {}


def _unit(t):
    key = (str(t.device), t.dtype)
    one = _units.get(key)
    if one is None:
        one = _units[key] = torch.ones((), dtype=t.dtype, device=t.device)
    return one


def _leaf_grad(t):
    from ...functional import fanout_leftover
    left = fanout_leftover(t)
    if left is None:
        return t.grad
    return left if t.grad is None else t.grad + left


class lean_capture:
    _stream = None

    def __init__(self, graph, pool=None):
        self.graph, self.pool = graph, pool

    def __enter__(self):
        if lean_capture._stream is None:
            lean_capture._stream = torch.cuda.Stream()
        self.stream = lean_capture._stream
        self.stream.wait_stream(torch.cuda.current_stream())
        self.ctx = torch.cuda.stream(self.stream)
        self.ctx.__enter__()
        kw = {"pool": self.pool} if self.pool is not None else {}
        self.graph.capture_begin(capture_error_mode="thread_local", **kw)

    def __exit__(self, *exc):
        self.graph.capture_end()
        self.ctx.__exit__(*exc)
        torch.cuda.current_stream().wait_stream(self.stream)
        return False


_GRAPH_DUMP = __import__("os").environ.get("OMNI_GRAPH_DUMP", "")


def make_side_stream(device=None):
    import ctypes
    import os
    n = int(os.environ.get("OMNI_SIDE_CUS", str(SIDE_CUS_DEFAULT)))
    prio = int(os.environ.get("OMNI_SIDE_PRIORITY", "0"))
    if 0 < n < 256:
        hip = ctypes.CDLL("libamdhip64.so")
        dev = torch.cuda.current_device() if device is None else torch.device(device).index
        with torch.cuda.device(dev):
            words = (ctypes.c_uint32 * 8)()
            for bit in range(n):
                words[bit // 32] |= 1 << (bit % 32)
            st = ctypes.c_void_p()
            rc = hip.hipExtStreamCreateWithCUMask(ctypes.byref(st), 8, words)
            if rc == 0 and st.value:
                _MASKED_STREAMS.append(st)
                return torch.cuda.ExternalStream(st.value, device=dev)
    if prio != 0:
        return torch.cuda.Stream(priority=prio)
    return torch.cuda.Stream()


SIDE_CUS_DEFAULT = 0
POOL_CUT = __import__("os").environ.get("OMNI_PIPE_POOL_CUT", "1") != "0"
_PIPE_TIMING = __import__("os").environ.get("OMNI_PIPE_TIMING", "0") == "1"


def set_pipe_timing(flag):
    global _PIPE_TIMING
    _PIPE_TIMING = bool(flag)


def pipe_timing_report(graphed, last=10):
    torch.cuda.synchronize()
    recs = graphed._timing[-last:]
    if not recs:
        return ""
    n = len(recs[0]["m"])
    out = []
    for k in range(n):
        m = sum(r["t0"].elapsed_time(r["m"][k]) for r in recs) / len(recs)
        w = [r["t0"].elapsed_time(r["w"][k]) for r in recs if r["w"][k] is not None]
        x = [r["t0"].elapsed_time(r["x"][k]) for r in recs if r.get("x") and r["x"][k] is not None]
        out.append("M%d end %.3f ms%s%s" % (k, m, (", W%d end %.3f ms" % (k, sum(w) / len(w))) if w else "",
                                            (", X%d end %.3f ms" % (k, sum(x) / len(x))) if x else ""))
    host = {}
    for r in recs:
        for name, us in r["host"]:
            host.setdefault(name, []).append(us)
    out.append("host us per launch: " + ", ".join("%s %.0f" % (k, sum(v) / len(v)) for k, v in host.items()))
    return " | ".join(out)


def pipe_timing_table(graphed, last=10):
    torch.cuda.synchronize()
# ... 52 lines not shown
        from ...kernels import detmode
        detmode.prewarm(torch.cuda.current_device())
        prev_mode = HF.side_mode()
        HF.side_mode("inline")
        try:
            ga, gb = torch.cuda.CUDAGraph(), torch.cuda.CUDAGraph()
            with torch.cuda.graph(ga, capture_error_mode="thread_local"):
                self.losses, self.total = self._phase_a()
            with torch.cuda.graph(gb, pool=ga.pool(), capture_error_mode="thread_local"):
                self._phase_b()
        finally:
            HF.side_mode(prev_mode)
        self.graph_a, self.graph_b = ga, gb

    def _phase_a(self):
        self.optimizer.zero_grad()
        losses = self.model(self.static_batch, self.static_packed)
        total = total_loss(losses)
        total.backward(_unit(total))
        return losses, total.detach()

    def _phase_b(self):
        self.cut.backward()

    def __call__(self):
        if self.graph_a is not None:
            self.graph_a.replay()
        else:
            self.losses, self.total = self._phase_a()
        pending = self.optimizer.all_reduce_begin("early", self.group)
        if self.graph_b is not None:
            self.graph_b.replay()
        else:
            self._phase_b()
        pending += self.optimizer.all_reduce_begin("late", self.group)
        return self.losses, self.total, pending


class GraphedForwardBackward:
    def __init__(self, model, optimizer, batch, packed, warmup=3):
        assert torch.cuda.is_available(), "hipGraph capture needs the GPU"
        self.model, self.optimizer = model, optimizer
        self.static_batch, self.static_packed = batch, packed
        side = torch.cuda.Stream()
        side.wait_stream(torch.cuda.current_stream())
        with torch.cuda.stream(side):
            for _ in range(warmup):
                self._body()
        torch.cuda.current_stream().wait_stream(side)
        torch.cuda.synchronize()
        self.graph = torch.cuda.CUDAGraph()
        from ... import functional as HF
        from ...kernels import detmode
        detmode.prewarm(torch.cuda.current_device())
        prev_mode = HF.side_mode()
        HF.side_mode("inline")
        try:
            with torch.cuda.graph(self.graph, capture_error_mode="thread_local"):
                self.losses, self.total = self._body()
        finally:
            HF.side_mode(prev_mode)

    def _body(self):
        self.optimizer.zero_grad()
        losses = self.model(self.static_batch, self.static_packed)
        total = total_loss(losses)
        total.backward(_unit(total))
        return losses, total.detach()

    def __call__(self):
        self.graph.replay()
        return self.losses, self.total


class StageCuts:

    def __init__(self):
        self.cuts = []

    def __len__(self):
        return len(self.cuts)

    def __call__(self, x):
        from ...functional import fanout
        if isinstance(x, dict):
            dst = {k: fanout(v.detach().requires_grad_(True)) for k, v in x.items()}
        elif isinstance(x, (tuple, list)):
            dst = tuple(None if v is None else fanout(v.detach().requires_grad_(True)) for v in x)
        else:
            dst = fanout(x.detach().requires_grad_(True))
        self.cuts.append([x, dst, []])
        return dst

    def attach_root(self, loss):
        self.cuts[-1][2].append(loss)

    def reset(self):
        self.cuts.clear()

    def backward_last(self):
        src, dst, roots = self.cuts.pop()
        if isinstance(src, dict):
            pairs = [(src[k], _leaf_grad(dst[k])) for k in src]
        elif isinstance(src, (tuple, list)):
            pairs = [(a, _leaf_grad(b)) for a, b in zip(src, dst) if a is not None]
        else:
            pairs = [(src, _leaf_grad(dst))]
        pairs = [p for p in pairs if p[1] is not None]
        del src, dst
        if pairs or roots:
            torch.autograd.backward([p[0] for p in pairs] + list(roots), [p[1] for p in pairs] + [_unit(r) for r in roots])


class GraphedPipelined:

    _warm_stream = None

    def __init__(self, model, optimizer, batch, packed, warmup=3, graphs=True, group=None, pools=None):
        from ... import functional as HF
        self.HF = HF
        self.model, self.optimizer, self.group = model, optimizer, group
        self.static_batch, self.static_packed = batch, packed
        self.pools = pools
        self.cuts = StageCuts()
        self._install()
        bottom_up = getattr(getattr(model, "backbone", None), "bottom_up", None)
        if bottom_up is not None and hasattr(type(bottom_up), "stage_cut"):
            import os
            if os.environ.get("OMNI_PIPE_CUTS") is not None:
                bottom_up.stage_cut_at = tuple(x for x in os.environ["OMNI_PIPE_CUTS"].split(",") if x)
        self.stages = None
        self._timing = []
        if not graphs:
            return
        assert torch.cuda.is_available(), "hipGraph capture needs the GPU"
        self.side = make_side_stream()
        prev_mode = HF.side_mode()
        HF.side_mode("inline")
        if GraphedPipelined._warm_stream is None:
            GraphedPipelined._warm_stream = torch.cuda.Stream()
        warm = GraphedPipelined._warm_stream
        warm.wait_stream(torch.cuda.current_stream())
        import time as _time
        _t0 = _time.perf_counter()
        muted = getattr(self.optimizer, "_exchange_muted", False)
        self.optimizer._exchange_muted = True
        try:
            with torch.cuda.stream(warm):
                for _ in range(warmup):
                    _, _, pending = self._eager()
                    assert not pending
                    del pending
        finally:
            self.optimizer._exchange_muted = muted
        torch.cuda.current_stream().wait_stream(warm)
        torch.cuda.synchronize()
        _t1 = _time.perf_counter()
        HF.side_mode("collect")
        from ...kernels import detmode, wino
        detmode.prewarm(torch.cuda.current_device())
        try:
            stages = []
            pool_m, pool_w = self.pools if self.pools is not None else (None, None)
            self._held = []
            self.prologue = None
            while True:
                if not stages and self._split_labels():
                    gm, pool_w = self._capture_stage0_labels(pool_m, pool_w)
                else:
                    gm = torch.cuda.CUDAGraph()
                    if _GRAPH_DUMP:
                        gm.enable_debug_mode()
                    with lean_capture(gm, pool_m), detmode.domain("M"):
# ... 228 lines not shown
```

omni3d_amd/functional.py:

```python
import torch
from torch.autograd import Function
from os import environ as _environ

_os_environ_get = _environ.get

from .kernels import glue
from .kernels import bnpool, conv, det, wino

CL = torch.channels_last


def _cl(t):
    return t if t.is_contiguous(memory_format=CL) else t.contiguous(memory_format=CL)


def _direct_grad(t):
    if t is not None and getattr(t, "_omni_direct_grad", False) and t.grad is not None and t.requires_grad:
        return t.grad
    return None


def _parts_out(parts, like):
    return parts if parts is not None else like.new_zeros((0, 1))


_FANOUT = _os_environ_get("OMNI_FANOUT", "1") != "0"


class _GradSlot:
    __slots__ = ("buf", "remaining")

    def __init__(self):
        self.buf, self.remaining = None, 0


def fanout(t):
    if _FANOUT and t.requires_grad and torch.is_grad_enabled() and getattr(t, "_omni_slot", None) is None:
        slot = t._omni_slot = _GradSlot()
        if t.grad_fn is not None:
            nr = t.output_nr

            def hand_over(grads):
                left = fanout_leftover(slot)
                if left is None:
                    return None
                if grads[nr] is None:
                    raise RuntimeError(f"omni3d_amd.functional.fanout: a consumer of a {tuple(left.shape)} activation registered with its "
                                       "gradient fan-in slot in forward but never ran in backward (its output does not reach the loss), and "
                                       "no other gradient arrived that the withheld sum could be added to.  Feed that consumer a detached "
                                       "input, or set OMNI_FANOUT=0.")
                grads = list(grads)
                grads[nr] = grads[nr] + left
                return tuple(grads)
            t.grad_fn.register_prehook(hand_over)
    return t


def fanout_leftover(t_or_slot):
    slot = t_or_slot if isinstance(t_or_slot, _GradSlot) else getattr(t_or_slot, "_omni_slot", None)
    if slot is None or slot.buf is None:
        return None
    left, slot.buf, slot.remaining = slot.buf, None, 0
    return left


def _slot_enter(t, needs_grad):
    slot = getattr(t, "_omni_slot", None) if (needs_grad and t is not None) else None
    if slot is not None:
        slot.remaining += 1
    return slot


def _slot_deliver(slot, compute):
    if slot is None:
        return compute(None)
    out = compute(slot.buf)
    slot.remaining -= 1
    if slot.remaining <= 0:
        slot.buf = None
        return out
    slot.buf = out
    return None


def _add_carry(out, carry):
    return out if carry is None else out + carry


def _carry_pitch(c):
    N, C, H, W = c.shape
    sn, sc, sh, sw = c.stride()
    if c.dtype != torch.float32 or sc != 1 or sw < C or (sw & 3) or (c.data_ptr() & 15) or (c.storage_offset() & 3):
        return None
    if (H > 1 and sh != W * sw) or (N > 1 and sn != H * W * sw):
        return None
    return sw


_side = {"mode": "stream" if _os_environ_get("OMNI_WGRAD_STREAM", "1") != "0" else "inline",
         "batch": int(_os_environ_get("OMNI_WGRAD_BATCH", "8")), "streams": {}, "pending": [], "queue": [], "main": None}


def side_mode(mode=None):
    if mode is not None:
        assert mode in ("inline", "stream", "collect")
        side_join()
        _side["mode"] = mode
    return _side["mode"]


def side_take():
    q, keep = list(_side["queue"]), list(_side["pending"])
    _side["queue"].clear()
    _side["pending"].clear()
    return q, keep


def _side_flush():
    if not _side["queue"]:
        return
    main, st = _side["main"]
    st.wait_stream(main)
    with torch.cuda.stream(st), wino.batched_wgrads():
        for fn in _side["queue"]:
            fn()
    _side["queue"].clear()


def _side_run(fn, keepalive):
    dev = keepalive[0].device
    mode = _side["mode"]
    if mode == "inline" or (dev.type != "cuda" and mode != "collect"):
        return fn()
    _side["queue"].append(fn)
    _side["pending"].extend(keepalive)
    if mode == "collect":
        return None
    if _side["main"] is None:
        st = _side["streams"].get(dev.index)
        if st is None:
            st = _side["streams"][dev.index] = torch.cuda.Stream(device=dev)
        _side["main"] = (torch.cuda.current_stream(dev), st)
        torch.autograd.Variable._execution_engine.queue_callback(side_join)
    if len(_side["queue"]) >= _side["batch"]:
        _side_flush()
    return None


BIAS_GRAD_SIDE = _environ.get("OMNI_BIAS_GRAD_SIDE", "1") != "0"


def _bias_grad(dy2d, gb):
    if gb is None or not BIAS_GRAD_SIDE:
        return bnpool.bias_grad(dy2d, accum_into=gb)
    return _side_run(lambda: bnpool.bias_grad(dy2d, accum_into=gb), (dy2d,))


def side_join():
    if _side["mode"] == "collect":
        return
    if _side["main"] is not None:
        _side_flush()
        main, st = _side["main"]
        main.wait_stream(st)
        _side["main"] = None
# ... 310 lines not shown
        dy = _cl(dy)
        dx = conv.dwconv_dgrad(dy, w, (x.shape[2], x.shape[3]), stride, pad) if ctx.needs_input_grad[0] else None
        dw = conv.dwconv_wgrad(x, dy, w.shape[2], stride, pad).contiguous() if ctx.needs_input_grad[1] else None
        return dx, dw, None, None


def depthwise_conv2d(x, w, stride=1, pad=1):
    return _DepthwiseConv2d.apply(x, w, stride, pad)


class _Linear(Function):
    @staticmethod
    def forward(ctx, x, w, bias, relu, w_grad_view=None, b_grad_view=None):
        gw = _direct_grad(w) if w_grad_view is None else w_grad_view
        ctx.direct = (gw if (gw is not None and gw.is_contiguous()) else None, _direct_grad(bias) if b_grad_view is None else b_grad_view)
        x, w = x.contiguous(), w.contiguous()
        y = conv.linear_fwd(x, w, bias, relu)
        ctx.save_for_backward(x, w, y if relu else None)
        ctx.cfg = (relu, bias is not None)
        return y

    @staticmethod
    def backward(ctx, dy):
        x, w, y = ctx.saved_tensors
        relu, has_bias = ctx.cfg
        dy = dy.contiguous()
        if relu:
            dy = bnpool.relu_bwd(dy, y)
        gw, gb = ctx.direct
        dx = conv.linear_dgrad(dy, w) if ctx.needs_input_grad[0] else None
        dw = None
        if ctx.needs_input_grad[1]:
            dw = _side_run(lambda: conv.linear_wgrad(x, dy, accum_into=gw), (x, dy)) if gw is not None else conv.linear_wgrad(x, dy)
        db = _bias_grad(dy, gb) if (has_bias and ctx.needs_input_grad[2]) else None
        return dx, dw, db, None, None, None


def linear(x, w, bias=None, relu=False, w_grad_view=None, b_grad_view=None):
    return _Linear.apply(x, w, bias, relu, w_grad_view, b_grad_view)


def fused_linear(x, weights, biases, rows, relu=False):
    from .cubercnn.solver.build import fused_view
    cols = weights[0].shape[1]
    training = torch.is_grad_enabled() and any(w.requires_grad for w in weights)
    fw, fb = fused_view(weights, training), fused_view(biases, training)
    if fw is not None and fb is not None and fw[0].numel() == rows * cols and fb[0].numel() == rows:
        w, b = fw[0].view(rows, cols), fb[0]
        if training:
            return _Linear.apply(x, w.detach().requires_grad_(True), b.detach().requires_grad_(True), relu, fw[1].view(rows, cols), fb[1])
        return _Linear.apply(x, w, b, relu, None, None)
    pad = rows - sum(w.shape[0] for w in weights)
    w = torch.cat(list(weights) + ([weights[0].new_zeros(pad, cols)] if pad else []), dim=0)
    b = torch.cat(list(biases) + ([biases[0].new_zeros(pad)] if pad else []), dim=0)
    return _Linear.apply(x, w, b, relu, None, None)


_BN_REMASK = _os_environ_get("OMNI_BN_REMASK", "1") != "0"
_BN_BWD_FUSE = _os_environ_get("OMNI_BN_BWD_FUSE", "1") != "0"


class _BatchNorm(Function):
    @staticmethod
    def forward(ctx, x, gamma, beta, running_mean, running_var, residual, relu, eps, momentum, partials=None):
        gg, gb = _direct_grad(gamma), _direct_grad(beta)
        ctx.direct = (gg, gb) if (gg is not None and gb is not None) else None
        ctx.res_slot = _slot_enter(residual, residual is not None and ctx.needs_input_grad[5])
        x = _cl(x)
        res = _cl(residual) if residual is not None else None
        y, mean_rstd, scale_shift = bnpool.bn_fwd(x, gamma, beta, running_mean, running_var, res, relu, eps, momentum, partials)
        remask = relu and residual is None and _BN_REMASK
        ctx.save_for_backward(x, gamma, mean_rstd, (y if relu and not remask else None), (scale_shift if remask else None))
        ctx.cfg = (relu, residual is not None)
        if _BN_BWD_FUSE and residual is None and (remask or not relu):
            y._omni_bn_below = (x, mean_rstd, scale_shift if relu else None)
        return y

    @staticmethod
    def backward(ctx, dy):
        x, gamma, mean_rstd, y, scale_shift = ctx.saved_tensors
        relu, has_res = ctx.cfg
        parts = getattr(dy, "_omni_bn_bwd_parts", None)
        if parts is not None:
            parts = parts[0] if parts[1].data_ptr() == mean_rstd.data_ptr() and dy.is_contiguous(memory_format=CL) else None
        want_dres = has_res and ctx.needs_input_grad[5]
        box = []

        dyk = dy if (parts is None and not dy.is_contiguous(memory_format=CL) and _carry_pitch(dy) is not None) else _cl(dy)

        def run(carry):
            ok = carry is not None and parts is None and _carry_pitch(carry) is not None
            dx_, dres_, dgamma_, dbeta_ = bnpool.bn_bwd(x, dyk, y, gamma, mean_rstd, relu, want_dres=want_dres, accum_into=ctx.direct,
                                                        scale_shift=scale_shift, partials=parts, res_carry=carry if ok else None)
            box.append((dx_, dgamma_, dbeta_))
            return dres_ if (ok or carry is None) else dres_ + carry

        dres = _slot_deliver(ctx.res_slot, run) if want_dres else run(None)
        dx, dgamma, dbeta = box[0]
        return dx, dgamma, dbeta, None, None, dres, None, None, None, None


def batch_norm_train(x, gamma, beta, running_mean, running_var, residual=None, relu=False, eps=1e-5, momentum=0.1):
    return _BatchNorm.apply(x, gamma, beta, running_mean, running_var, residual, relu, eps, momentum, getattr(x, "_omni_bn_partials", None))


class _FrozenBatchNorm(Function):

    @staticmethod
    def forward(ctx, x, gamma, beta, running_mean, running_var, residual, relu, eps):
        gg, gb = _direct_grad(gamma), _direct_grad(beta)
        ctx.direct = (gg, gb) if (gg is not None and gb is not None) else None
        ctx.res_slot = _slot_enter(residual, residual is not None and ctx.needs_input_grad[5])
        x = _cl(x)
        res = _cl(residual) if residual is not None else None
        y = bnpool.bn_frozen_fwd(x, gamma, beta, running_mean, running_var, res, relu, eps)
        remask = relu and residual is None and _BN_REMASK
        ctx.save_for_backward(x, gamma, beta, running_mean, running_var, (y if relu and not remask else None))
        ctx.cfg = (relu, residual is not None, remask, eps)
        return y

    @staticmethod
    def backward(ctx, dy):
        x, gamma, beta, running_mean, running_var, y = ctx.saved_tensors
        relu, has_res, remask, eps = ctx.cfg
        want_dres = has_res and ctx.needs_input_grad[5]
        params = ctx.needs_input_grad[1] or ctx.needs_input_grad[2]
        box = []
        dyk = dy if (not dy.is_contiguous(memory_format=CL) and _carry_pitch(dy) is not None) else _cl(dy)

        def run(carry):
            ok = carry is not None and _carry_pitch(carry) is not None
            dx_, dres_, dgamma_, dbeta_ = bnpool.bn_frozen_bwd(x, dyk, y, gamma, beta, running_mean, running_var, eps, relu, remask,
                                                               want_dres=want_dres, param_grads=params,
                                                               accum_into=ctx.direct if params else None, res_carry=carry if ok else None)
            box.append((dx_, dgamma_, dbeta_))
            return dres_ if (ok or carry is None) else dres_ + carry

        dres = _slot_deliver(ctx.res_slot, run) if want_dres else run(None)
        dx, dgamma, dbeta = box[0]
        return dx, dgamma, dbeta, None, None, dres, None, None


def batch_norm_frozen(x, gamma, beta, running_mean, running_var, residual=None, relu=False, eps=1e-5):
    return _FrozenBatchNorm.apply(x, gamma, beta, running_mean, running_var, residual, relu, eps)


class _MaxPool2(Function):
    @staticmethod
    def forward(ctx, x):
        ctx.slot = _slot_enter(x, ctx.needs_input_grad[0])
        x = _cl(x)
        ctx.save_for_backward(x)
        return bnpool.maxpool2_fwd(x)

    @staticmethod
    def backward(ctx, dy):
        (x,) = ctx.saved_tensors

        dyk = dy if (not dy.is_contiguous(memory_format=CL) and _carry_pitch(dy) is not None) else _cl(dy)

        def run(carry):
            if carry is not None and (_carry_pitch(carry) is None or (x.shape[2] | x.shape[3]) & 1):
                return bnpool.maxpool2_bwd(x, dyk) + carry
            return bnpool.maxpool2_bwd(x, dyk, carry=carry)
        return _slot_deliver(ctx.slot, run)


class _AvgPool2(Function):
    @staticmethod
    def forward(ctx, x):
        x = _cl(x)
        ctx.hw = (x.shape[2], x.shape[3])
        return bnpool.avgpool2_fwd(x)

    @staticmethod
    def backward(ctx, dy):
        return bnpool.avgpool2_bwd(_cl(dy), ctx.hw)


class _Subsample2(Function):
    @staticmethod
    def forward(ctx, x):
        ctx.slot = _slot_enter(x, ctx.needs_input_grad[0])
        x = _cl(x)
        ctx.hw = (x.shape[2], x.shape[3])
        return bnpool.subsample2_fwd(x)

    @staticmethod
    def backward(ctx, dy):
        def run(carry):
            if carry is not None and _carry_pitch(carry) is None:
                return bnpool.subsample2_bwd(_cl(dy), ctx.hw) + carry
            return bnpool.subsample2_bwd(_cl(dy), ctx.hw, carry=carry)
        return _slot_deliver(ctx.slot, run)


class _Upsample2Add(Function):
    @staticmethod
    def forward(ctx, lat, top):
        ctx.slot = _slot_enter(top, ctx.needs_input_grad[1])
        return bnpool.upsample2_add(_cl(lat), _cl(top))

    @staticmethod
    def backward(ctx, dout):
        dout = _cl(dout)

        def run(carry):
            if carry is not None and _carry_pitch(carry) is None:
                return bnpool.upsample2_bwd(dout) + carry
            return bnpool.upsample2_bwd(dout, carry=carry)
        return dout, _slot_deliver(ctx.slot, run)


class _CatChannels(Function):

    @staticmethod
    def forward(ctx, *xs):
        ctx.slots = [_slot_enter(x, ctx.needs_input_grad[i]) for i, x in enumerate(xs)]
        ctx.sizes = [x.shape[1] for x in xs]
        return torch.cat(xs, 1)

    @staticmethod
    def backward(ctx, g):
        outs, off = [], 0
        for i, (slot, c) in enumerate(zip(ctx.slots, ctx.sizes)):
            piece = g[:, off:off + c]
            off += c
            outs.append(_slot_deliver(slot, lambda carry, piece=piece: _add_carry(piece, carry)) if ctx.needs_input_grad[i] else None)
        return tuple(outs)


class _CatConv1x1(Function):

    @staticmethod
    def forward(ctx, w, want_stats, *xs):
        ctx.set_materialize_grads(False)
        ctx.direct = _direct_grad(w)
        ctx.slots = [_slot_enter(x, ctx.needs_input_grad[2 + i]) for i, x in enumerate(xs)]
        xs = [_cl(x) for x in xs]
        w = _cl(w)
        y, parts = conv.conv1x1_multi_fwd(xs, w, want_stats=want_stats)
        ctx.save_for_backward(w, *xs)
        parts = _parts_out(parts, y)
        ctx.mark_non_differentiable(parts)
        return y, parts

# ... 388 lines not shown
```

omni3d_amd/kernels/bnpool.py:

```python
import os

import torch

from .. import lib as _lib
from .conv import _nhwc


def _like_cl(shape_nhwc, ref):
    return torch.empty(shape_nhwc, dtype=torch.float32, device=ref.device)


FUSE_ROWS = int(os.environ.get("OMNI_BN_FUSE_ROWS", "512"))


def _pitched_out(out, N, H, W, C):
    assert tuple(out.shape) == (N, C, H, W) and out.dtype == torch.float32 and out.stride(1) == 1, (out.shape, out.stride())
    ldy = out.stride(3)
    assert out.stride(2) == W * ldy and out.stride(0) == H * W * ldy and ldy >= C and ldy % 4 == 0 and out.data_ptr() % 16 == 0
    return out, out.data_ptr(), ldy


def bn_fwd(x, gamma, beta, running_mean, running_var, residual=None, relu=False, eps=1e-5, momentum=0.1, partials=None, out=None):
    xv = _nhwc(x)
    rv = _nhwc(residual) if residual is not None else None
# ... 20 lines not shown
def bn_apply(x, scale_shift, residual=None, relu=False):
    xv = _nhwc(x)
    rv = _nhwc(residual) if residual is not None else None
    N, H, W, C = xv.shape
    L = _lib.check_device(xv, rv, scale_shift)
    y = _like_cl((N, H, W, C), x)
    L.call("omni_bn_apply", _lib.ptr(xv), _lib.ptr(scale_shift), _lib.ptr(rv), _lib.ptr(y), N * H * W, C, int(relu),
           _lib.stream_of(x))
    return y.permute(0, 3, 1, 2)


def bn_frozen_fwd(x, gamma, beta, running_mean, running_var, residual=None, relu=False, eps=1e-5):
    xv = _nhwc(x)
    rv = _nhwc(residual) if residual is not None else None
    N, H, W, C = xv.shape
    L = _lib.check_device(xv, rv, gamma, beta, running_mean, running_var)
    for t in (gamma, beta, running_mean, running_var):
        assert t.dtype == torch.float32 and t.is_contiguous() and t.numel() == C
    y = _like_cl((N, H, W, C), x)
    L.call("omni_bn_frozen_fwd", _lib.ptr(xv), _lib.ptr(gamma), _lib.ptr(beta), _lib.ptr(running_mean), _lib.ptr(running_var), float(eps),
           _lib.ptr(rv), _lib.ptr(y), N * H * W, C, int(relu), _lib.stream_of(x))
    return y.permute(0, 3, 1, 2)


def bn_frozen_bwd(x, dy, y, gamma, beta, running_mean, running_var, eps=1e-5, relu=False, remask=False, want_dres=False, param_grads=True,
                  accum_into=None, res_carry=None):
    xv = _nhwc(x)
    N, H, W, C = xv.shape
    dy_pitched = not dy.is_contiguous(memory_format=torch.channels_last)
    if dy_pitched:
        assert tuple(dy.shape) == tuple(x.shape) and dy.stride(1) == 1
    dyv = None if dy_pitched else _nhwc(dy)
    mode = 0
    yv = None
    if relu:
        mode = 2 if remask else 1
        yv = None if remask else _nhwc(y)
    L = _lib.check_device(xv, dyv, yv, gamma, beta, running_mean, running_var)
    dx = _like_cl((N, H, W, C), x)
    dres = _like_cl((N, H, W, C), x) if want_dres else None
    if res_carry is not None:
        assert want_dres and tuple(res_carry.shape) == tuple(x.shape)
    dgamma = dbeta = ws = None
    if param_grads:
        if accum_into is not None:
            dgamma, dbeta = accum_into
            assert dgamma.is_contiguous() and dbeta.is_contiguous() and dgamma.numel() == C and dbeta.numel() == C
        else:
            dgamma = torch.empty(C, dtype=torch.float32, device=x.device)
            dbeta = torch.empty(C, dtype=torch.float32, device=x.device)
        ws = torch.empty(2 * C * 512, dtype=torch.float32, device=x.device)
    L.call("omni_bn_frozen_bwd", _lib.ptr(xv), dy.data_ptr() if dy_pitched else _lib.ptr(dyv), dy.stride(3) if dy_pitched else C, _lib.ptr(yv),
           _lib.ptr(gamma), _lib.ptr(beta), _lib.ptr(running_mean), _lib.ptr(running_var), float(eps), _lib.ptr(dx), _lib.ptr(dres),
           _lib.ptr(res_carry), res_carry.stride(3) if res_carry is not None else 0, _lib.ptr(dgamma), _lib.ptr(dbeta), _lib.ptr(ws),
           ws.numel() if ws is not None else 0, N * H * W, C, mode, int(accum_into is not None), _lib.stream_of(x))
    if accum_into is not None:
        dgamma = dbeta = None
    return dx.permute(0, 3, 1, 2), (dres.permute(0, 3, 1, 2) if want_dres else None), dgamma, dbeta


def bn_bwd(x, dy, y, gamma, mean_rstd, relu=False, want_dres=False, accum_into=None, scale_shift=None, partials=None, res_carry=None):
    xv = _nhwc(x)
    dy_pitched = not dy.is_contiguous(memory_format=torch.channels_last)
    dyv = None if dy_pitched else _nhwc(dy)
    mode = int(bool(relu))
    if relu and scale_shift is not None:
        assert y is None and scale_shift.is_contiguous() and scale_shift.numel() == 2 * xv.shape[3]
        yv, mode = scale_shift, 2
    else:
        yv = _nhwc(y) if relu else None
    N, H, W, C = xv.shape
    L = _lib.check_device(xv, dyv, yv, gamma, mean_rstd)
    dx = _like_cl((N, H, W, C), x)
    dres = _like_cl((N, H, W, C), x) if want_dres else None
    if accum_into is not None:
        dgamma, dbeta = accum_into
        assert dgamma.is_contiguous() and dbeta.is_contiguous()
    else:
        dgamma = torch.empty(C, dtype=torch.float32, device=x.device)
        dbeta = torch.empty(C, dtype=torch.float32, device=x.device)
    coef = torch.empty(3 * C, dtype=torch.float32, device=x.device)
    ws = None
    if partials is not None:
        assert partials.is_contiguous() and partials.shape[1] == 2 * C and res_carry is None and not dy_pitched
    else:
        ws = torch.empty(2 * C * 258, dtype=torch.float64, device=x.device)
    if res_carry is not None or dy_pitched:
        assert tuple(dy.shape) == tuple(x.shape) and dy.stride(1) == 1
        if res_carry is not None:
            assert want_dres and tuple(res_carry.shape) == tuple(x.shape)
    L.call("omni_bn_bwd_algo", _lib.ptr(xv), dy.data_ptr() if dy_pitched else _lib.ptr(dyv), dy.stride(3) if dy_pitched else C, _lib.ptr(yv),
           _lib.ptr(gamma), _lib.ptr(mean_rstd), _lib.ptr(partials), partials.shape[0] if partials is not None else 0, _lib.ptr(dx),
           _lib.ptr(dres), _lib.ptr(res_carry), res_carry.stride(3) if res_carry is not None else 0, _lib.ptr(dgamma), _lib.ptr(dbeta),
           _lib.ptr(ws), _lib.ptr(coef), N * H * W, C, mode, int(accum_into is not None), FUSE_ROWS, _lib.stream_of(x))
    if accum_into is not None:
        dgamma = dbeta = None
    return dx.permute(0, 3, 1, 2), (dres.permute(0, 3, 1, 2) if want_dres else None), dgamma, dbeta


def _simple(name, src, out_shape, dims, extra_in=()):
    L = _lib.check_device(src, *extra_in)
    out = torch.empty(out_shape, dtype=torch.float32, device=src.device)
    L.call(name, *[_lib.ptr(t) for t in (src, *extra_in)], _lib.ptr(out), *dims, _lib.stream_of(src))
    return out


def maxpool2_fwd(x):
    xv = _nhwc(x)
    N, H, W, C = xv.shape
    return _simple("omni_maxpool2_fwd", xv, (N, H // 2, W // 2, C), (N, H, W, C)).permute(0, 3, 1, 2)


def maxpool2_bwd(x, dy, carry=None):
    xv = _nhwc(x)
    N, H, W, C = xv.shape
    if carry is None and dy.is_contiguous(memory_format=torch.channels_last):
        return _simple("omni_maxpool2_bwd", xv, (N, H, W, C), (N, H, W, C), extra_in=(_nhwc(dy),)).permute(0, 3, 1, 2)
    assert (carry is None or tuple(carry.shape) == tuple(x.shape)) and tuple(dy.shape) == (N, C, H // 2, W // 2) and dy.stride(1) == 1
    L = _lib.check_device(xv)
    dx = torch.empty((N, H, W, C), dtype=torch.float32, device=x.device)
    L.call("omni_maxpool2_bwd_carry", _lib.ptr(xv), dy.data_ptr(), dy.stride(3), _lib.ptr(carry), carry.stride(3) if carry is not None else 0,
           _lib.ptr(dx), N, H, W, C, _lib.stream_of(x))
    return dx.permute(0, 3, 1, 2)


def avgpool2_fwd(x):
    xv = _nhwc(x)
    N, H, W, C = xv.shape
    return _simple("omni_avgpool2_fwd", xv, (N, H // 2, W // 2, C), (N, H, W, C)).permute(0, 3, 1, 2)


def avgpool2_bwd(dy, in_hw):
    dyv = _nhwc(dy)
    N, _, _, C = dyv.shape
    H, W = in_hw
    return _simple("omni_avgpool2_bwd", dyv, (N, H, W, C), (N, H, W, C)).permute(0, 3, 1, 2)


def subsample2_fwd(x):
    xv = _nhwc(x)
    N, H, W, C = xv.shape
    return _simple("omni_subsample2_fwd", xv, (N, (H - 1) // 2 + 1, (W - 1) // 2 + 1, C), (N, H, W, C)).permute(0, 3, 1, 2)


def subsample2_bwd(dy, in_hw, carry=None):
    dyv = _nhwc(dy)
    N, _, _, C = dyv.shape
    H, W = in_hw
    if carry is None:
        return _simple("omni_subsample2_bwd", dyv, (N, H, W, C), (N, H, W, C)).permute(0, 3, 1, 2)
    assert tuple(carry.shape) == (N, C, H, W)
    L = _lib.check_device(dyv)
    dx = torch.empty((N, H, W, C), dtype=torch.float32, device=dy.device)
    L.call("omni_subsample2_bwd_carry", _lib.ptr(dyv), carry.data_ptr(), carry.stride(3), _lib.ptr(dx), N, H, W, C, _lib.stream_of(dy))
    return dx.permute(0, 3, 1, 2)


def upsample2_add(lat, top):
    lv, tv = _nhwc(lat), _nhwc(top)
    N, H, W, C = lv.shape
    assert tv.shape == (N, H // 2, W // 2, C), (tv.shape, lv.shape)
    return _simple("omni_upsample2_add", lv, (N, H, W, C), (N, H, W, C), extra_in=(tv,)).permute(0, 3, 1, 2)


def upsample2_bwd(dout, carry=None):
    dv = _nhwc(dout)
    N, H, W, C = dv.shape
    if carry is None:
        return _simple("omni_upsample2_bwd", dv, (N, H // 2, W // 2, C), (N, H, W, C)).permute(0, 3, 1, 2)
    assert tuple(carry.shape) == (N, C, H // 2, W // 2)
    L = _lib.check_device(dv)
    dtop = torch.empty((N, H // 2, W // 2, C), dtype=torch.float32, device=dout.device)
    L.call("omni_upsample2_bwd_carry", _lib.ptr(dv), carry.data_ptr(), carry.stride(3), _lib.ptr(dtop), N, H, W, C, _lib.stream_of(dout))
    return dtop.permute(0, 3, 1, 2)


def preprocess(images_u8, pixel_mean, pixel_std, size_divisibility=0, image_hw=None):
    assert images_u8.dtype == torch.uint8 and images_u8.dim() == 4 and images_u8.shape[1] == 3
    images_u8 = images_u8.contiguous()
    N, _, H, W = images_u8.shape
    PH, PW = H, W
    if size_divisibility > 1:
        s = size_divisibility
        PH, PW = (H + s - 1) // s * s, (W + s - 1) // s * s
    L = _lib.check_device(images_u8)
    out = torch.empty((N, PH, PW, 4), dtype=torch.float32, device=images_u8.device)
    m, s = [float(v) for v in pixel_mean], [float(v) for v in pixel_std]
    if image_hw is not None:
        assert image_hw.dtype == torch.int32 and tuple(image_hw.shape) == (N, 2) and image_hw.is_contiguous()
        L.call("omni_preprocess_masked", _lib.ptr(images_u8), _lib.ptr(image_hw), _lib.ptr(out), N, H, W, PH, PW, m[0], m[1], m[2], s[0], s[1],
               s[2], _lib.stream_of(images_u8))
    else:
        L.call("omni_preprocess", _lib.ptr(images_u8), _lib.ptr(out), N, H, W, PH, PW, m[0], m[1], m[2], s[0], s[1], s[2],
               _lib.stream_of(images_u8))
    return out.permute(0, 3, 1, 2)


def preprocess_list(images, pixel_mean, pixel_std, size_divisibility=0, image_hw=None):
    import ctypes
    N = len(images)
    if not (0 < N <= 64):
        return None
    H, W = images[0].shape[-2:]
    for im in images:
        if im.dtype != torch.uint8 or im.dim() != 3 or tuple(im.shape) != (3, H, W) or not im.is_contiguous() or im.device != images[0].device:
            return None
# ... 46 lines not shown
```

omni3d_amd/kernels/conv.py:

```python
import os

import torch

from .. import lib as _lib
from . import detmode as _det


def _nhwc(t):
    if t.dim() != 4:
        raise ValueError("expected a 4-D tensor")
    v = t.permute(0, 2, 3, 1)
    if not v.is_contiguous():
        v = v.contiguous()
    return v


def to_channels_last(t):
    return t.contiguous(memory_format=torch.channels_last)


def _fwd_launch(L, x, w, bias, out, N, H, W, C, K, R, S, stride, pad, ldx, ldo, relu, tile, splits, like, stats=None, stats_rows=0, nblk_addr=None):
    if _det.on():
        _det.plan_launch(L, "omni_conv2d_fwd_det", like, (x, w, bias, out, N, H, W, C, K, R, S, stride, pad, ldx, ldo, int(relu)),
                         ask=(tile, splits), late=(_lib.ptr(stats), stats_rows, nblk_addr))
# ... 230 lines not shown


def linear_wgrad(x, dy, accum_into=None):
    M, C = x.shape
    K = dy.shape[1]
    L = _lib.check_device(x, dy)
    if accum_into is not None:
        assert accum_into.is_contiguous() and accum_into.shape == (K, C)
        _wgrad_launch(L, _lib.ptr(x), _lib.ptr(dy), _lib.ptr(accum_into), M, 1, 1, C, K, 1, 1, 1, 0, C, K, 1, 0, x)
        return None
    dw = torch.empty((K, C), dtype=torch.float32, device=x.device)
    _wgrad_launch(L, _lib.ptr(x), _lib.ptr(dy), _lib.ptr(dw), M, 1, 1, C, K, 1, 1, 1, 0, C, K, 0, 0, x)
    return dw


def stem_eligible(x_shape, w_shape, stride, pad):
    K, C, R, S = w_shape
    return K == 16 and R == S and stride == 1 and pad == R // 2 and (C, R) in ((4, 7), (16, 3)) and x_shape[1] == C


def stem_conv_fwd(x, w):
    xv, wv = _nhwc(x), _nhwc(w)
    N, H, W, C = xv.shape
    K, R = wv.shape[0], wv.shape[1]
    L = _lib.check_device(xv, wv)
    out = torch.empty((N, H, W, K), dtype=torch.float32, device=x.device)
    L.call("omni_stem_conv_fwd", _lib.ptr(xv), _lib.ptr(wv), _lib.ptr(out), N, H, W, C, K, R, C, K, _lib.stream_of(x))
    return out.permute(0, 3, 1, 2)


def stem_first_eligible(x_shape, w):
    return (_det.on() and tuple(w.shape) == (16, 3, 7, 7) and x_shape[1] == 4 and w.is_contiguous(memory_format=torch.channels_last)
            and w.dtype == torch.float32)


def stem_first_fwd(x, w, want_stats):
    xv = _nhwc(x)
    wv = w.permute(0, 2, 3, 1)
    assert wv.is_contiguous()
    N, H, W, C = xv.shape
    L = _lib.check_device(xv, wv)
    out = torch.empty((N, H, W, 16), dtype=torch.float32, device=x.device)
    stats = _stats_buf(16, x.device) if want_stats else None
    cell, addr = _nblk_cell()
    L.call("omni_stem_conv_fwd_cw", _lib.ptr(xv), _lib.ptr(wv), 3, _lib.ptr(out), N, H, W, C, 16, 7, C, 16, _lib.ptr(stats),
           STATS_ROWS if want_stats else 0, addr, _lib.stream_of(x))
    return out.permute(0, 3, 1, 2), (stats[:cell.value] if want_stats and cell.value > 0 else None)


def stem_first_wgrad(x, dy, accum_into=None):
    xv, dv = _nhwc(x), _nhwc(dy)
    N, H, W, C = xv.shape
    L = _lib.check_device(xv, dv)
    dst = accum_into.permute(0, 2, 3, 1) if accum_into is not None else torch.empty((16, 7, 7, 3), dtype=torch.float32, device=x.device)
    assert dst.is_contiguous() and tuple(dst.shape) == (16, 7, 7, 3)
    acc = int(accum_into is not None)
    _det.plan_launch(L, "omni_stem_conv_wgrad_det_cw", x, (_lib.ptr(xv), _lib.ptr(dv), _lib.ptr(dst), 3, N, H, W, C, 16, 7, C, 16, acc),
                     counters=False)
    return None if accum_into is not None else dst.permute(0, 3, 1, 2)


_STEM_DGRAD = os.environ.get("OMNI_STEM_DGRAD", "1") != "0"


def stem_dgrad_eligible(x_shape, w_shape, stride, pad):
    K, C, R, S = w_shape
    if not _STEM_DGRAD or R != 3 or S != 3 or pad != 1 or C != 16 or x_shape[1] != 16:
        return False
    return (stride == 1 and K == 16) or (stride == 2 and K == 32)


def stem_conv_dgrad(dy, w, in_hw, stride):
    dyv, wv = _nhwc(dy), _nhwc(w)
    N, OH, OW, K = dyv.shape
    H, W = in_hw
    assert (OH, OW) == ((H - 1) // stride + 1, (W - 1) // stride + 1) and tuple(wv.shape) == (K, 3, 3, 16)
    L = _lib.check_device(dyv, wv)
    dx = torch.empty((N, H, W, 16), dtype=torch.float32, device=dy.device)
    L.call("omni_stem_conv_dgrad" if stride == 1 else "omni_stem_conv_s2_dgrad", _lib.ptr(dyv), _lib.ptr(wv), _lib.ptr(dx), N, H, W, 16, K, 3,
           K, 16, _lib.stream_of(dy))
    return dx.permute(0, 3, 1, 2)


_STEM_WGRAD_ALL = os.environ.get("OMNI_STEM_WGRAD_ALL", "1") != "0"


def stem_wgrad_eligible(x_shape, w_shape, stride, pad):
    K, C, R, S = w_shape
    if R != S or pad != R // 2 or x_shape[1] != C:
        return False
    if stride == 1:
        return K == 16 and ((C, R) == (16, 3) or ((C, R) == (4, 7) and _det.on() and _STEM_WGRAD_ALL))
    return _STEM_WGRAD_ALL and stride == 2 and (K, C, R) == (32, 16, 3) and x_shape[2] % 2 == 0 and x_shape[3] % 2 == 0


def stem_conv_wgrad(x, dy, R, accum_into=None, stride=1):
    xv, dv = _nhwc(x), _nhwc(dy)
    N, H, W, C = xv.shape
    K = dv.shape[3]
    L = _lib.check_device(xv, dv)
    on = _det.on()
    if accum_into is not None:
        dst = accum_into.permute(0, 2, 3, 1)
        assert dst.is_contiguous() and tuple(dst.shape) == (K, R, R, C)
    else:
        dst = torch.empty((K, R, R, C), dtype=torch.float32, device=x.device)
    head = (_lib.ptr(xv), _lib.ptr(dv), _lib.ptr(dst), N, H, W, C, K, R, C, K, int(accum_into is not None))
    if stride == 2:
        name, head = "omni_stem_conv_s2_wgrad", head + (int(on),)
    else:
        name = "omni_stem_conv_wgrad_det" if on else "omni_stem_conv_wgrad"
    if on:
        _det.plan_launch(L, name, x, head, counters=False)
    elif stride == 2:
        L.call(name, *head, None, 0, None, _lib.stream_of(x))
    else:
        L.call(name, *head, _lib.stream_of(x))
    return None if accum_into is not None else dst.permute(0, 3, 1, 2)


def _taps(w):
    C, _, R, S = w.shape
    return w.reshape(C, R, S).permute(1, 2, 0).contiguous()


def dwconv_fwd(x, w, stride=1, pad=1):
    xv, wt = _nhwc(x), _taps(w)
    N, H, W, C = xv.shape
    R = wt.shape[0]
    OH, OW = (H + 2 * pad - R) // stride + 1, (W + 2 * pad - R) // stride + 1
    L = _lib.check_device(xv, wt)
    out = torch.empty((N, OH, OW, C), dtype=torch.float32, device=x.device)
    L.call("omni_dwconv_fwd", _lib.ptr(xv), _lib.ptr(wt), _lib.ptr(out), N, H, W, C, R, stride, pad, _lib.stream_of(x))
    return out.permute(0, 3, 1, 2)


def dwconv_dgrad(dy, w, in_hw, stride=1, pad=1):
    dyv, wt = _nhwc(dy), _taps(w)
    N, _, _, C = dyv.shape
    H, W = in_hw
    L = _lib.check_device(dyv, wt)
    dx = torch.empty((N, H, W, C), dtype=torch.float32, device=dy.device)
    L.call("omni_dwconv_dgrad", _lib.ptr(dyv), _lib.ptr(wt), _lib.ptr(dx), N, H, W, C, wt.shape[0], stride, pad, _lib.stream_of(dy))
    return dx.permute(0, 3, 1, 2)


def dwconv_wgrad(x, dy, R, stride=1, pad=1):
    xv, dyv = _nhwc(x), _nhwc(dy)
    N, H, W, C = xv.shape
    L = _lib.check_device(xv, dyv)
    dw = torch.empty((R, R, C), dtype=torch.float32, device=x.device)
    L.call("omni_dwconv_wgrad", _lib.ptr(xv), _lib.ptr(dyv), _lib.ptr(dw), N, H, W, C, R, stride, pad, _lib.stream_of(x))
    return dw.permute(2, 0, 1).reshape(C, 1, R, R)


def grouped_conv2d_fwd(x, w, groups, stride=1, pad=0):
    xv, wv = _nhwc(x), _nhwc(w)
    N, H, W, C = xv.shape
    K, R, S, Cg = wv.shape
    assert Cg * groups == C, (C, Cg, groups)
    OH, OW = (H + 2 * pad - R) // stride + 1, (W + 2 * pad - S) // stride + 1
    L = _lib.check_device(xv, wv)
    out = torch.empty((N, OH, OW, K), dtype=torch.float32, device=x.device)
    L.call("omni_grouped_conv2d_fwd", _lib.ptr(xv), _lib.ptr(wv), _lib.ptr(out), N, H, W, C, K, R, S, stride, pad, groups, _lib.stream_of(x))
    return out.permute(0, 3, 1, 2)

# ... 23 lines not shown
```

omni3d_amd/kernels/wino.py:

```python
import torch

from .. import lib as _lib
from . import detmode as _det

CL = torch.channels_last


import os as _os

_F43 = _os.environ.get("OMNI_WINOGRAD_F43", "1") != "0"
_F43_MIN_TILES = int(_os.environ.get("OMNI_WINOGRAD_F43_MIN_TILES", "256"))


_MIN_TILES = int(_os.environ.get("OMNI_WINO_MIN_TILES", "256"))
_DGRAD_MIN_TILES = int(_os.environ.get("OMNI_WINO_DGRAD_MIN_TILES", "256"))


def eligible(x_shape, w_shape, stride, pad):
    N, C, H, W = x_shape
    K, _, R, S = w_shape
    if not (R == 3 and S == 3 and stride == 1 and pad == 1 and H % 2 == 0 and W % 2 == 0 and C % 32 == 0 and K % 32 == 0):
        return False
    if C >= 128 and K >= 128 and N * (H // 2) * (W // 2) >= _MIN_TILES:
        return True
# ... 228 lines not shown
    tile = 2 if Mt.shape[0] == 16 else 4
    N, H, W = shape
    K = Mt.shape[2]
    xv = bn_x.permute(0, 2, 3, 1)
    assert xv.is_contiguous() and tuple(xv.shape) == (N, H, W, K)
    L = _lib.check_device(Mt, xv, mean_rstd, scale_shift)
    y = torch.empty((N, H, W, K), dtype=torch.float32, device=Mt.device)
    stats = _stats_buf(K, Mt.device)
    cell, addr = _nblk_cell()
    L.call("omni_wino_out_bn_bwd_stats", _lib.ptr(Mt), _lib.ptr(y), N, H, W, K, tile, _lib.ptr(xv), _lib.ptr(mean_rstd), _lib.ptr(scale_shift),
           _lib.ptr(stats), STATS_ROWS, addr, _lib.stream_of(Mt))
    return y.permute(0, 3, 1, 2), (stats[:cell.value] if cell.value > 0 else None)


def transform_dy(dy, tile=2):
    dv = _nhwc(dy)
    N, H, W, K = dv.shape
    L = _lib.check_device(dv)
    dM = torch.empty((_points(tile), N * (H // tile) * (W // tile), K), dtype=torch.float32, device=dy.device)
    L.call("omni_wino_dy", _lib.ptr(dv), _lib.ptr(dM), N, H, W, K, tile, _lib.stream_of(dy))
    return dM


def transform_dy_both(dy, tile=2):
    dv = _nhwc(dy)
    N, H, W, K = dv.shape
    L = _lib.check_device(dv)
    shape = (_points(tile), N * (H // tile) * (W // tile), K)
    dM = torch.empty(shape, dtype=torch.float32, device=dy.device)
    Vd = torch.empty(shape, dtype=torch.float32, device=dy.device)
    L.call("omni_wino_dy_in", _lib.ptr(dv), _lib.ptr(dM), _lib.ptr(Vd), N, H, W, K, tile, _lib.stream_of(dy))
    return dM, Vd


def transform_dweights(dU, accum_into=None):
    P, K, C = dU.shape
    tile = 2 if P == 16 else 4
    L = _lib.check_device(dU)
    if accum_into is not None:
        gv = accum_into.permute(0, 2, 3, 1)
        assert gv.is_contiguous()
        L.call("omni_wino_dweights", _lib.ptr(dU), _lib.ptr(gv), K, C, 1, tile, _lib.stream_of(dU))
        return None
    dw = torch.empty((K, 3, 3, C), dtype=torch.float32, device=dU.device)
    L.call("omni_wino_dweights", _lib.ptr(dU), _lib.ptr(dw), K, C, 0, tile, _lib.stream_of(dU))
    return dw.permute(0, 3, 1, 2)


def conv3x3_fwd(x, w, bias=None, relu=False, U=None, tile=2, want_stats=False):
    N, _, H, W = x.shape
    V = transform_input(x, tile)
    if U is None:
        U = transform_weights(w, tile=tile)[0]
    Mt = gemm_batched(V, U)
    if want_stats:
        y, parts = transform_output_stats(Mt, (N, H, W))
        return y, V, parts
    return transform_output(Mt, (N, H, W), bias, relu), V


def conv3x3_dgrad(dy, w, U_flip=None, tile=2, carry=None):
    N, _, H, W = dy.shape
    if U_flip is None:
        U_flip = transform_weights(w, want_u=False, want_flip=True, tile=tile)[1]
    Mt = gemm_batched(transform_input(dy, tile), U_flip)
    return transform_output(Mt, (N, H, W), carry=carry)


def conv3x3_backward(V, dy, w, U_flip, accum_into=None, side_run=None, bn_below=None, carry=None):
    N, _, H, W = dy.shape
    tile = 2 if V.shape[0] == 16 else 4
    dM, Vd = transform_dy_both(dy, tile)
    if side_run is not None and accum_into is not None:
        dw = side_run(lambda: wgrad_into(V, dM, accum_into), (V, dM))
    else:
        dw = None
    if U_flip is None:
        U_flip = transform_weights(w, want_u=False, want_flip=True, tile=tile)[1]
    if carry is not None:
        dx = transform_output(gemm_batched(Vd, U_flip), (N, H, W), carry=carry)
    elif bn_below is not None and tile == 4:
        dx, parts = transform_output_bn_bwd(gemm_batched(Vd, U_flip), (N, H, W), *bn_below[:3])
        if parts is not None:
            dx._omni_bn_bwd_parts = (parts, bn_below[1])
    else:
        dx = transform_output(gemm_batched(Vd, U_flip), (N, H, W))
    if side_run is None or accum_into is None:
        dw = transform_dweights(gemm_batched_wgrad(V, dM), accum_into)
    return dx, dw


def conv3x3_wgrad(V, dy, accum_into=None):
    dM = transform_dy(dy, 2 if V.shape[0] == 16 else 4)
    if accum_into is not None:
        return wgrad_into(V, dM, accum_into)
    return transform_dweights(gemm_batched_wgrad(V, dM), None)
```

Before: 379.8 images/s.

## Fuse BN-backward channel reductions into maxpool and stem dgrad backward kernels

Extends the existing trick of computing batch-norm backward partial sums inside the producer of dy to the maxpool backward and stem conv data-gradient kernels. The per-channel sum(g) and sum(g*xhat) partials are then handed to the BN backward, which can skip its own reduction pass over x and dy. The partials are also propagated across graph cut points, guarded by version and pointer checks, and allowed alongside a residual carry. The risks are extra loads of the BN input inside the producer kernels, a capped grid when stats are collected, and fragile attribute plumbing on gradient tensors.

```diff
diff --git a/include/omni3d_hip.h b/include/omni3d_hip.h
--- a/include/omni3d_hip.h
+++ b/include/omni3d_hip.h
@@ -266,6 +266,12 @@
 int omni_bn_bwd_partials(const float* x, const float* dy, const float* y, const float* gamma, const float* mean_rstd,
                          const float* partial, int nblk, float* dx, float* dres, float* dgamma, float* dbeta, float* coef,
                          int P, int C, int relu, int accumulate_param_grads, void* stream);
+int omni_stem_conv_dgrad_bn_bwd_stats(const float* dy, const float* w, float* dx, int N, int H, int W, int C, int K, int R, int stride,
+                                      int lddy, int lddx, const float* bn_x, const float* mean_rstd, const float* scale_shift,
+                                      const float* bn_y, float* stats, int stats_rows, int* nblk_out, void* stream);
+int omni_maxpool2_bwd_bn_bwd_stats(const float* x, const float* dy, long long lddy, const float* carry, long long ldc, float* dx, int N,
+                                   int H, int W, int C, const float* bn_x, const float* mean_rstd, int relu, float* stats, int stats_rows,
+                                   int* nblk_out, void* stream);
 int omni_stem_conv_fwd_stats(const float* x, const float* w, float* out, int N, int H, int W, int C, int K, int R, int ldx,
                              int ldo, float* stats, int stats_rows, int* nblk_out, void* stream);
 int omni_bn_fwd_partials(const float* x, const float* partial, int nblk, const float* gamma, const float* beta,
diff --git a/omni3d_amd/csrc/bn_bwd_stats.h b/omni3d_amd/csrc/bn_bwd_stats.h
--- /dev/null
+++ b/omni3d_amd/csrc/bn_bwd_stats.h
@@ -0,0 +1,82 @@
+#pragma once
+#include <device_rt.h>
+
+struct BnBwdStats {
+    const float* x;
+    const float* mean_rstd;
+    const float* scale_shift;
+    const float* y;
+};
+
+struct BnBwdCoef4 {
+    float4 mu, rs, sc, sh;
+};
+__device__ __forceinline__ BnBwdCoef4 bn_bwd_coef4(const BnBwdStats& b, int K, int kc) {
+    const float4 z = make_float4(0.f, 0.f, 0.f, 0.f);
+    BnBwdCoef4 c{z, z, z, z};
+    if (b.x != nullptr) {
+        c.mu = *reinterpret_cast<const float4*>(b.mean_rstd + kc);
+        c.rs = *reinterpret_cast<const float4*>(b.mean_rstd + K + kc);
+        if (b.y == nullptr && b.scale_shift != nullptr) {
+            c.sc = *reinterpret_cast<const float4*>(b.scale_shift + kc);
+            c.sh = *reinterpret_cast<const float4*>(b.scale_shift + K + kc);
+        }
+    }
+    return c;
+}
+__device__ __forceinline__ float4 bn_bwd_mask4(float4 g, float4 y) {
+    return make_float4(y.x > 0.f ? g.x : 0.f, y.y > 0.f ? g.y : 0.f, y.z > 0.f ? g.z : 0.f, y.w > 0.f ? g.w : 0.f);
+}
+__device__ __forceinline__ void bn_bwd_acc4(const BnBwdStats& b, const BnBwdCoef4& c, float4 g, float4 xv, float4 yv, float4& sv, float4& sq) {
+    if (b.y != nullptr) g = bn_bwd_mask4(g, yv);
+    else if (b.scale_shift != nullptr) g = bn_bwd_mask4(g, xv * c.sc + c.sh);
+    const float4 xh = (xv - c.mu) * c.rs;
+    sv = sv + g;
+    sq = sq + g * xh;
+}
+
+__device__ __forceinline__ void block_channel_stats(float4 sv, float4 sq, int K, float* __restrict__ stats) {
+    __shared__ float4 r0[256], r1[256];
+    const int K4 = K >> 2, t = threadIdx.x;
+    r0[t] = sv;
+    r1[t] = sq;
+    __syncthreads();
+    if (t < K4) {
+        float4 a = r0[t], b = r1[t];
+        for (int q = t + K4; q < 256; q += K4) {
+            a = make_float4(a.x + r0[q].x, a.y + r0[q].y, a.z + r0[q].z, a.w + r0[q].w);
+            b = make_float4(b.x + r1[q].x, b.y + r1[q].y, b.z + r1[q].z, b.w + r1[q].w);
+        }
+        *reinterpret_cast<float4*>(stats + (long)blockIdx.x * 2 * K + 4 * t) = a;
+        *reinterpret_cast<float4*>(stats + (long)blockIdx.x * 2 * K + K + 4 * t) = b;
+    }
+}
+
+struct BnBwdCoef1 {
+    float mu, rs, sc, sh;
+};
+__device__ __forceinline__ BnBwdCoef1 bn_bwd_coef1(const BnBwdStats& b, int K, int k) {
+    BnBwdCoef1 c{0.f, 0.f, 0.f, 0.f};
+    if (b.x != nullptr) {
+        c.mu = b.mean_rstd[k];
+        c.rs = b.mean_rstd[K + k];
+        if (b.y == nullptr && b.scale_shift != nullptr) { c.sc = b.scale_shift[k]; c.sh = b.scale_shift[K + k]; }
+    }
+    return c;
+}
+__device__ __forceinline__ void bn_bwd_acc1(const BnBwdStats& b, const BnBwdCoef1& c, float g, long off, float& sv, float& sq) {
+    const float xv = b.x[off];
+    if (b.y != nullptr) g = b.y[off] > 0.f ? g : 0.f;
+    else if (b.scale_shift != nullptr) g = xv * c.sc + c.sh > 0.f ? g : 0.f;
+    sv += g;
+    sq += g * ((xv - c.mu) * c.rs);
+}
+__device__ __forceinline__ void bn_bwd_row16(float sv, float sq, float* __restrict__ s, float* __restrict__ row) {
+    const int tid = threadIdx.x, lane = tid & 63, wave = tid >> 6;
+    sv += __shfl_xor(sv, 16, 64); sq += __shfl_xor(sq, 16, 64);
+    sv += __shfl_xor(sv, 32, 64); sq += __shfl_xor(sq, 32, 64);
+    __syncthreads();
+    if (lane < 16) { s[wave * 32 + lane] = sv; s[wave * 32 + 16 + lane] = sq; }
+    __syncthreads();
+    if (tid < 32) row[tid] = s[tid] + s[32 + tid] + s[64 + tid] + s[96 + tid];
+}
diff --git a/omni3d_amd/csrc/bn_pool.hip b/omni3d_amd/csrc/bn_pool.hip
--- a/omni3d_amd/csrc/bn_pool.hip
+++ b/omni3d_amd/csrc/bn_pool.hip
@@ -1,4 +1,5 @@
 #include <device_rt.h>
+#include "bn_bwd_stats.h"
 
 namespace {
 
@@ -562,9 +563,12 @@
 
 __global__ void __launch_bounds__(256) maxpool2_bwd_kernel(const float* __restrict__ x, const float* __restrict__ dy,
                                                            float* __restrict__ dx, int N, int H, int W, int C,
-                                                           const float* __restrict__ carry, long ldc, long lddy) {
+                                                           const float* __restrict__ carry, long ldc, long lddy,
+                                                           float* __restrict__ stats, BnBwdStats bnb) {
     const int C4 = C >> 2, OH = H >> 1, OW = W >> 1;
     const long total = (long)N * OH * OW * C4;
+    const BnBwdCoef4 cf = bn_bwd_coef4(bnb, C, 4 * (int)(threadIdx.x % C4));
+    float4 sv = f4(0.f), sq = f4(0.f);
     for (long i = (long)blockIdx.x * blockDim.x + threadIdx.x; i < total; i += (long)gridDim.x * blockDim.x) {
         const int col = (int)(i % C4);
         long q = i / C4;
@@ -585,7 +589,15 @@
             d10 = d10 + ld4(carry + pc + (long)W * ldc); d11 = d11 + ld4(carry + pc + (long)W * ldc + ldc);
         }
         st4(dx + o, d00); st4(dx + o + C, d01); st4(dx + o + (long)W * C, d10); st4(dx + o + (long)W * C + C, d11);
-    }
+        if (bnb.x != nullptr) {
+            const float4 b00 = ld4(bnb.x + o), b01 = ld4(bnb.x + o + C), b10 = ld4(bnb.x + o + (long)W * C), b11 = ld4(bnb.x + o + (long)W * C + C);
+            bn_bwd_acc4(bnb, cf, d00, b00, v00, sv, sq);
+            bn_bwd_acc4(bnb, cf, d01, b01, v01, sv, sq);
+            bn_bwd_acc4(bnb, cf, d10, b10, v10, sv, sq);
+            bn_bwd_acc4(bnb, cf, d11, b11, v11, sv, sq);
+        }
+    }
+    if (stats != nullptr) block_channel_stats(sv, sq, C, stats);
 }
 
 template <int DIR>
@@ -814,7 +826,7 @@
     if (P <= 0 || C <= 0 || (C & 3) || C > 4096 || relu < 0 || relu > 2 || (relu && y == nullptr)) return OMNI_ERR_ARG;
     if (lddy == 0) lddy = C;
     if (bad_carry(res_carry, ldc, C) || (res_carry != nullptr && dres == nullptr) || bad_carry(dy, lddy, C)) return OMNI_ERR_ARG;
-    if ((partial != nullptr && (nblk <= 0 || res_carry != nullptr || lddy != C)) || (partial == nullptr && ws == nullptr)) return OMNI_ERR_ARG;
+    if ((partial != nullptr && (nblk <= 0 || lddy != C)) || (partial == nullptr && ws == nullptr)) return OMNI_ERR_ARG;
     hipStream_t st = (hipStream_t)stream;
     if (partial == nullptr) {
         nblk = red_grid(P, C);
@@ -900,16 +912,39 @@
     return omni_launch_status();
 }
 
-int omni_maxpool2_bwd_carry(const float* x, const float* dy, long long lddy, const float* carry, long long ldc, float* dx, int N, int H,
-                            int W, int C, void* stream) {
+static int maxpool2_bwd_impl(const float* x, const float* dy, long long lddy, const float* carry, long long ldc, float* dx, int N, int H,
+                             int W, int C, float* stats, int stats_rows, int* nblk_out, BnBwdStats bnb, void* stream) {
+    if (nblk_out) *nblk_out = 0;
     if ((C & 3) || H < 2 || W < 2 || bad_carry(carry, ldc, C) || (carry != nullptr && ((H & 1) || (W & 1))) || bad_carry(dy, lddy, C))
         return OMNI_ERR_ARG;
     const long total = (long)N * (H / 2) * (W / 2) * (C / 4);
     if (total == 0) return OMNI_OK;
     if ((H & 1) || (W & 1)) omni_memset_async(dx, 0, sizeof(float) * (size_t)N * H * W * C, (hipStream_t)stream);
-    hipLaunchKernelGGL(maxpool2_bwd_kernel, dim3(ew_grid(total)), dim3(256), 0, (hipStream_t)stream, x, dy, dx, N, H, W, C, carry, (long)ldc,
-                       (long)lddy);
-    return omni_launch_status();
+    int grid = ew_grid(total);
+    const int rows = stats_rows < BN_FUSE_ROWS_DEFAULT ? stats_rows : BN_FUSE_ROWS_DEFAULT;
+    const bool st = stats != nullptr && bnb.x != nullptr && !((H | W) & 1) && C <= 1024 && (256 % (C / 4)) == 0 && rows >= 1;
+    if (st) {
+        if (grid > rows) grid = rows;
+        if (nblk_out) *nblk_out = grid;
+    } else {
+        bnb.x = nullptr;
+    }
+    hipLaunchKernelGGL(maxpool2_bwd_kernel, dim3(grid), dim3(256), 0, (hipStream_t)stream, x, dy, dx, N, H, W, C, carry, (long)ldc,
+                       (long)lddy, st ? stats : (float*)nullptr, bnb);
+    return omni_launch_status();
+}
+
+int omni_maxpool2_bwd_carry(const float* x, const float* dy, long long lddy, const float* carry, long long ldc, float* dx, int N, int H,
+                            int W, int C, void* stream) {
+    return maxpool2_bwd_impl(x, dy, lddy, carry, ldc, dx, N, H, W, C, nullptr, 0, nullptr, BnBwdStats{nullptr, nullptr, nullptr, nullptr}, stream);
+}
+
+int omni_maxpool2_bwd_bn_bwd_stats(const float* x, const float* dy, long long lddy, const float* carry, long long ldc, float* dx, int N,
+                                   int H, int W, int C, const float* bn_x, const float* mean_rstd, int relu, float* stats, int stats_rows,
+                                   int* nblk_out, void* stream) {
+    if (bn_x == nullptr || mean_rstd == nullptr || stats == nullptr || nblk_out == nullptr) return OMNI_ERR_ARG;
+    return maxpool2_bwd_impl(x, dy, lddy, carry, ldc, dx, N, H, W, C, stats, stats_rows, nblk_out,
+                             BnBwdStats{bn_x, mean_rstd, nullptr, relu ? x : nullptr}, stream);
 }
 
 int omni_maxpool2_bwd(const float* x, const float* dy, float* dx, int N, int H, int W, int C, void* stream) {
diff --git a/omni3d_amd/csrc/stem_conv.hip b/omni3d_amd/csrc/stem_conv.hip
--- a/omni3d_amd/csrc/stem_conv.hip
+++ b/omni3d_amd/csrc/stem_conv.hip
@@ -1,4 +1,5 @@
 #include <device_rt.h>
+#include "bn_bwd_stats.h"
 
 namespace {
 
@@ -7,7 +8,7 @@
 template <int C, int R, bool ROT = false>
 __global__ void __launch_bounds__(256) stem_conv_fwd_kernel(const float* __restrict__ x, const float* __restrict__ w,
                                                             float* __restrict__ out, int N, int H, int W, int ldx, int ldo,
-                                                            float* __restrict__ stats, int cw) {
+                                                            float* __restrict__ stats, int cw, BnBwdStats bnb) {
     static_assert(!ROT || C == 16, "the rotated form is the 16 -> 16 layer's data gradient");
     constexpr int TH = 4, TW = 64, PAD = R / 2;
     constexpr int HR = TH + R - 1, HC = TW + R - 1 + (C == 4 ? 1 : 0);
@@ -110,6 +111,8 @@
             }
     }
     const int oy = oy0 + wave;
+    const bool bwd_stats = ROT && bnb.x != nullptr;
+    const BnBwdCoef1 cf = bn_bwd_coef1(bnb, 16, px);
     float sv = 0.f, sq = 0.f;
     if (oy < H) {
 #pragma unroll
@@ -118,27 +121,25 @@
             for (int i = 0; i < 4; ++i) {
                 const int ox = ox0 + 16 * b + 4 * g + i;
                 if (ox < W) {
-                    out[(((long)n * H + oy) * W + ox) * ldo + px] = acc[b][i];
-                    sv += acc[b][i];
-                    sq += acc[b][i] * acc[b][i];
+                    const long pix = ((long)n * H + oy) * W + ox;
+                    out[pix * ldo + px] = acc[b][i];
+                    if (bwd_stats) {
+                        bn_bwd_acc1(bnb, cf, acc[b][i], pix * 16 + px, sv, sq);
+                    } else {
+                        sv += acc[b][i];
+                        sq += acc[b][i] * acc[b][i];
+                    }
                 }
             }
     }
-    if (stats != nullptr) {
-        sv += __shfl_xor(sv, 16, 64); sq += __shfl_xor(sq, 16, 64);
-        sv += __shfl_xor(sv, 32, 64); sq += __shfl_xor(sq, 32, 64);
-        __syncthreads();
-        if (lane < 16) { s_in[wave * 32 + lane] = sv; s_in[wave * 32 + 16 + lane] = sq; }
-        __syncthreads();
-        if (tid < 32) stats[(long)blockIdx.x * 32 + tid] = s_in[tid] + s_in[32 + tid] + s_in[64 + tid] + s_in[96 + tid];
-    }
+    if (stats != nullptr) bn_bwd_row16(sv, sq, s_in, stats + (long)blockIdx.x * 32);
 }
 
 
 template <int C, int K>
 __global__ void __launch_bounds__(256) stem_dgrad_s2_kernel(const float* __restrict__ dy, const float* __restrict__ w,
                                                             float* __restrict__ dx, int N, int H, int W, int OH, int OW, int lddy,
-                                                            int lddx) {
+                                                            int lddx, float* __restrict__ stats, BnBwdStats bnb) {
     static_assert(C == 16 && K % 16 == 0, "N = 16 dx channels per MFMA block; dy channels in chunks of 16");
     constexpr int TH = 8, TW = 64, HR = TH / 2 + 1, HC = TW / 2 + 1, PP = K + 4, KP = K + 4, K4 = K / 4, KH = K / 16;
     __shared__ __attribute__((aligned(16))) float s_dy[HR * HC * PP];
@@ -185,6 +186,8 @@
     __syncthreads();
 
     const int px = lane & 15, g = lane >> 4;
+    const BnBwdCoef1 cf = bn_bwd_coef1(bnb, C, px);
+    float sv = 0.f, sq = 0.f;
 #pragma unroll 1
     for (int half = 0; half < 2; ++half) {
         const int y = half == 0 ? wave : TH - 1 - wave;
@@ -227,10 +230,14 @@
 #pragma unroll
                     for (int pw = 0; pw < 2; ++pw) {
                         const int iw = ox0 + 2 * (16 * b + 4 * g + i) + pw;
-                        if (iw < W) orow[(long)iw * lddx] = acc[pw][b][i];
-                    }
-        }
-    }
+                        if (iw < W) {
+                            orow[(long)iw * lddx] = acc[pw][b][i];
+                            if (bnb.x != nullptr) bn_bwd_acc1(bnb, cf, acc[pw][b][i], (((long)n * H + ih) * W + iw) * C + px, sv, sq);
+                        }
+                    }
+        }
+    }
+    if (stats != nullptr) bn_bwd_row16(sv, sq, s_dy, stats + (long)blockIdx.x * 32);
 }
 
 template <int C, int R, int S, int K>
@@ -394,9 +401,11 @@
 extern "C" {
 
 static int stem_fwd_impl(const float* x, const float* w, float* out, int N, int H, int W, int C, int K, int R, int ldx, int ldo,
-                         float* stats, int stats_rows, int* nblk_out, void* stream, bool rot = false, int cw = 0) {
+                         float* stats, int stats_rows, int* nblk_out, void* stream, bool rot = false, int cw = 0,
+                         BnBwdStats bnb = BnBwdStats{nullptr, nullptr, nullptr, nullptr}) {
     if (nblk_out) *nblk_out = 0;
     if (cw == 0) cw = C;
+    if (bnb.x != nullptr && (!rot || ldo != 16 || bnb.mean_rstd == nullptr)) return OMNI_ERR_ARG;
     if (N < 0 || H <= 0 || W <= 0 || K != 16 || ldx < C || ldo < K || (ldx & 3) || (rot && C != 16)) return OMNI_ERR_ARG;
     if (cw != C && (C != 4 || cw < 1 || cw > 4)) return OMNI_ERR_ARG;
     if (!((C == 4 && R == 7) || (C == 16 && R == 3))) return OMNI_ERR_ARG;
@@ -404,15 +413,16 @@
     const long tiles = (long)N * ((H + 3) / 4) * ((W + 63) / 64);
     float* sp = (stats != nullptr && tiles <= stats_rows) ? stats : nullptr;
     if (sp && nblk_out) *nblk_out = (int)tiles;
+    if (sp == nullptr) bnb.x = nullptr;
     if (C == 4)
         hipLaunchKernelGGL(HIP_KERNEL_NAME(stem_conv_fwd_kernel<4, 7>), dim3((unsigned)tiles), dim3(256), 0, (hipStream_t)stream, x, w,
-                           out, N, H, W, ldx, ldo, sp, cw);
+                           out, N, H, W, ldx, ldo, sp, cw, bnb);
     else if (rot)
         hipLaunchKernelGGL(HIP_KERNEL_NAME(stem_conv_fwd_kernel<16, 3, true>), dim3((unsigned)tiles), dim3(256), 0, (hipStream_t)stream, x, w,
-                           out, N, H, W, ldx, ldo, sp, cw);
+                           out, N, H, W, ldx, ldo, sp, cw, bnb);
     else
         hipLaunchKernelGGL(HIP_KERNEL_NAME(stem_conv_fwd_kernel<16, 3>), dim3((unsigned)tiles), dim3(256), 0, (hipStream_t)stream, x, w,
-                           out, N, H, W, ldx, ldo, sp, cw);
+                           out, N, H, W, ldx, ldo, sp, cw, bnb);
     return omni_launch_status();
 }
 
@@ -427,16 +437,36 @@
     return stem_fwd_impl(dy, w, dx, N, H, W, K, C, R, lddy, lddx, nullptr, 0, nullptr, stream, true);
 }
 
-int omni_stem_conv_s2_dgrad(const float* dy, const float* w, float* dx, int N, int H, int W, int C, int K, int R, int lddy, int lddx,
-                            void* stream) {
+static int stem_s2_dgrad_impl(const float* dy, const float* w, float* dx, int N, int H, int W, int C, int K, int R, int lddy, int lddx,
+                              float* stats, int stats_rows, int* nblk_out, BnBwdStats bnb, void* stream) {
+    if (nblk_out) *nblk_out = 0;
     if (N < 0 || H <= 0 || W <= 0 || C != 16 || K != 32 || R != 3 || lddy < K || lddx < C || (lddy & 3)) return OMNI_ERR_ARG;
+    if (bnb.x != nullptr && (lddx != C || bnb.mean_rstd == nullptr)) return OMNI_ERR_ARG;
     if (N == 0) return OMNI_OK;
     const int OH = (H - 1) / 2 + 1, OW = (W - 1) / 2 + 1;
     const long tiles = (long)N * ((H + 7) / 8) * ((W + 63) / 64);
     if (tiles > 0x7fffffff) return OMNI_ERR_ARG;
+    float* sp = (stats != nullptr && bnb.x != nullptr && tiles <= stats_rows) ? stats : nullptr;
+    if (sp && nblk_out) *nblk_out = (int)tiles;
+    if (sp == nullptr) bnb.x = nullptr;
     hipLaunchKernelGGL(HIP_KERNEL_NAME(stem_dgrad_s2_kernel<16, 32>), dim3((unsigned)tiles), dim3(256), 0, (hipStream_t)stream, dy, w, dx, N,
-                       H, W, OH, OW, lddy, lddx);
+                       H, W, OH, OW, lddy, lddx, sp, bnb);
     return omni_launch_status();
+}
+
+int omni_stem_conv_s2_dgrad(const float* dy, const float* w, float* dx, int N, int H, int W, int C, int K, int R, int lddy, int lddx,
+                            void* stream) {
+    return stem_s2_dgrad_impl(dy, w, dx, N, H, W, C, K, R, lddy, lddx, nullptr, 0, nullptr, BnBwdStats{nullptr, nullptr, nullptr, nullptr}, stream);
+}
+
+int omni_stem_conv_dgrad_bn_bwd_stats(const float* dy, const float* w, float* dx, int N, int H, int W, int C, int K, int R, int stride,
+                                      int lddy, int lddx, const float* bn_x, const float* mean_rstd, const float* scale_shift,
+                                      const float* bn_y, float* stats, int stats_rows, int* nblk_out, void* stream) {
+    if (bn_x == nullptr || mean_rstd == nullptr || stats == nullptr || nblk_out == nullptr) return OMNI_ERR_ARG;
+    const BnBwdStats bnb{bn_x, mean_rstd, scale_shift, bn_y};
+    if (stride == 2) return stem_s2_dgrad_impl(dy, w, dx, N, H, W, C, K, R, lddy, lddx, stats, stats_rows, nblk_out, bnb, stream);
+    if (stride != 1 || C != 16 || K != 16 || R != 3) return OMNI_ERR_ARG;
+    return stem_fwd_impl(dy, w, dx, N, H, W, K, C, R, lddy, lddx, stats, stats_rows, nblk_out, stream, true, 0, bnb);
 }
 
 int omni_stem_conv_fwd_stats(const float* x, const float* w, float* out, int N, int H, int W, int C, int K, int R, int ldx, int ldo,
diff --git a/omni3d_amd/csrc/winograd.hip b/omni3d_amd/csrc/winograd.hip
--- a/omni3d_amd/csrc/winograd.hip
+++ b/omni3d_amd/csrc/winograd.hip
@@ -1,4 +1,5 @@
 #include <device_rt.h>
+#include "bn_bwd_stats.h"
 
 namespace {
 
@@ -64,22 +65,6 @@
     }
 }
 
-__device__ __forceinline__ void block_channel_stats(float4 sv, float4 sq, int K, float* __restrict__ stats) {
-    __shared__ float4 r0[256], r1[256];
-    const int K4 = K >> 2, t = threadIdx.x;
-    r0[t] = sv;
-    r1[t] = sq;
-    __syncthreads();
-    if (t < K4) {
-        float4 a = r0[t], b = r1[t];
-        for (int q = t + K4; q < 256; q += K4) {
-            a = make_float4(a.x + r0[q].x, a.y + r0[q].y, a.z + r0[q].z, a.w + r0[q].w);
-            b = make_float4(b.x + r1[q].x, b.y + r1[q].y, b.z + r1[q].z, b.w + r1[q].w);
-        }
-        st4(stats + (long)blockIdx.x * 2 * K + 4 * t, a);
-        st4(stats + (long)blockIdx.x * 2 * K + K + 4 * t, b);
-    }
-}
 #define OMNI_ACC_STATS(v) do { sv = make_float4(sv.x + (v).x, sv.y + (v).y, sv.z + (v).z, sv.w + (v).w); \
                                sq = make_float4(sq.x + (v).x * (v).x, sq.y + (v).y * (v).y, sq.z + (v).z * (v).z, sq.w + (v).w * (v).w); } while (0)
 
@@ -382,11 +367,6 @@
     }
 }
 
-struct BnBwdStats {
-    const float* x;
-    const float* mean_rstd;
-    const float* scale_shift;
-};
 __global__ void __launch_bounds__(256) wino4_out_kernel(const float* __restrict__ M, const float* __restrict__ bias,
                                                         float* __restrict__ y, int N, int H, int W, int K, int relu,
                                                         float* __restrict__ stats, BnBwdStats bnb,
@@ -394,12 +374,7 @@
     const int K4 = K >> 2, TH = H >> 2, TW = W >> 2;
     const long T = (long)N * TH * TW, total = T * K4, plane = plane_in > 0 ? plane_in : T * K;
     float4 sv = z4(), sq = z4();
-    float4 mu = z4(), rs = z4(), sc = z4(), sh = z4();
-    if (bnb.x != nullptr) {
-        const int kc = 4 * (int)(threadIdx.x % K4);
-        mu = ld4(bnb.mean_rstd + kc); rs = ld4(bnb.mean_rstd + K + kc);
-        if (bnb.scale_shift != nullptr) { sc = ld4(bnb.scale_shift + kc); sh = ld4(bnb.scale_shift + K + kc); }
-    }
+    const BnBwdCoef4 cf = bn_bwd_coef4(bnb, K, 4 * (int)(threadIdx.x % K4));
     for (long i = (long)blockIdx.x * blockDim.x + threadIdx.x; i < total; i += (long)gridDim.x * blockDim.x) {
         const int k4 = (int)(i % K4);
         const long t = i / K4;
@@ -439,14 +414,7 @@
                 for (int c = 0; c < 4; ++c) {
                     const float4 v = row[c];
                     st4(o + (long)c * K, v);
-                    float4 g = v;
-                    if (bnb.scale_shift != nullptr) {
-                        const float4 yv = xv[c] * sc + sh;
-                        g = make_float4(yv.x > 0.f ? v.x : 0.f, yv.y > 0.f ? v.y : 0.f, yv.z > 0.f ? v.z : 0.f, yv.w > 0.f ? v.w : 0.f);
-                    }
-                    const float4 xh = (xv[c] - mu) * rs;
-                    sv = sv + g;
-                    sq = sq + g * xh;
+                    bn_bwd_acc4(bnb, cf, v, xv[c], z4(), sv, sq);
                 }
             } else {
 #pragma unroll
diff --git a/omni3d_amd/cubercnn/solver/graphed.py b/omni3d_amd/cubercnn/solver/graphed.py
--- a/omni3d_amd/cubercnn/solver/graphed.py
+++ b/omni3d_amd/cubercnn/solver/graphed.py
@@ -20,8 +20,28 @@
     from ...functional import fanout_leftover
     left = fanout_leftover(t)
     if left is None:
-        return t.grad
+        g, seen = t.grad, getattr(t, "_omni_cut_parts", None)
+        if g is not None and seen and seen[0] is not None:
+            parts, ptr = seen[0]
+            if g.data_ptr() == ptr and g._version == parts[2]:
+                g._omni_bn_bwd_parts = parts
+        return g
     return left if t.grad is None else t.grad + left
+
+
+def _cut_copy(v):
+    from ...functional import fanout
+    d = fanout(v.detach().requires_grad_(True))
+    below = getattr(v, "_omni_bn_below", None)
+    if below is not None:
+        d._omni_bn_below = below
+        seen = d._omni_cut_parts = [None]
+
+        def note(g, seen=seen):
+            parts = getattr(g, "_omni_bn_bwd_parts", None)
+            seen[0] = (parts, g.data_ptr()) if parts is not None and len(parts) > 2 else None
+        d.register_hook(note)
+    return d
 
 
 class lean_capture:
@@ -240,13 +260,12 @@
         return len(self.cuts)
 
     def __call__(self, x):
-        from ...functional import fanout
         if isinstance(x, dict):
-            dst = {k: fanout(v.detach().requires_grad_(True)) for k, v in x.items()}
+            dst = {k: _cut_copy(v) for k, v in x.items()}
         elif isinstance(x, (tuple, list)):
-            dst = tuple(None if v is None else fanout(v.detach().requires_grad_(True)) for v in x)
+            dst = tuple(None if v is None else _cut_copy(v) for v in x)
         else:
-            dst = fanout(x.detach().requires_grad_(True))
+            dst = _cut_copy(x)
         self.cuts.append([x, dst, []])
         return dst
 
diff --git a/omni3d_amd/functional.py b/omni3d_amd/functional.py
--- a/omni3d_amd/functional.py
+++ b/omni3d_amd/functional.py
@@ -81,6 +81,16 @@
         return out
     slot.buf = out
     return None
+
+
+def _slot_final(slot):
+    return slot is None or slot.remaining <= 1
+
+
+def _bn_parts_attach(dx, parts, bn_below):
+    if parts is not None:
+        dx._omni_bn_bwd_parts = (parts, bn_below[1], dx._version)
+    return dx
 
 
 def _add_carry(out, carry):
@@ -557,14 +567,15 @@
         relu, has_res = ctx.cfg
         parts = getattr(dy, "_omni_bn_bwd_parts", None)
         if parts is not None:
-            parts = parts[0] if parts[1].data_ptr() == mean_rstd.data_ptr() and dy.is_contiguous(memory_format=CL) else None
+            parts = parts[0] if (parts[1].data_ptr() == mean_rstd.data_ptr() and dy.is_contiguous(memory_format=CL)
+                                 and dy._version == parts[2]) else None
         want_dres = has_res and ctx.needs_input_grad[5]
         box = []
 
         dyk = dy if (parts is None and not dy.is_contiguous(memory_format=CL) and _carry_pitch(dy) is not None) else _cl(dy)
 
         def run(carry):
-            ok = carry is not None and parts is None and _carry_pitch(carry) is not None
+            ok = carry is not None and _carry_pitch(carry) is not None
             dx_, dres_, dgamma_, dbeta_ = bnpool.bn_bwd(x, dyk, y, gamma, mean_rstd, relu, want_dres=want_dres, accum_into=ctx.direct,
                                                         scale_shift=scale_shift, partials=parts, res_carry=carry if ok else None)
             box.append((dx_, dgamma_, dbeta_))
@@ -623,6 +634,7 @@
 class _MaxPool2(Function):
     @staticmethod
     def forward(ctx, x):
+        ctx.bn_below = getattr(x, "_omni_bn_below", None)
         ctx.slot = _slot_enter(x, ctx.needs_input_grad[0])
         x = _cl(x)
         ctx.save_for_backward(x)
@@ -634,9 +646,14 @@
 
         dyk = dy if (not dy.is_contiguous(memory_format=CL) and _carry_pitch(dy) is not None) else _cl(dy)
 
+        bn_below = ctx.bn_below if _slot_final(ctx.slot) else None
+
         def run(carry):
             if carry is not None and (_carry_pitch(carry) is None or (x.shape[2] | x.shape[3]) & 1):
                 return bnpool.maxpool2_bwd(x, dyk) + carry
+            if bn_below is not None and tuple(bn_below[0].shape) == tuple(x.shape):
+                dx_, parts_ = bnpool.maxpool2_bwd_bn_bwd(x, dyk, carry, bn_below[0], bn_below[1], bn_below[2] is not None)
+                return _bn_parts_attach(dx_, parts_, bn_below)
             return bnpool.maxpool2_bwd(x, dyk, carry=carry)
         return _slot_deliver(ctx.slot, run)
 
diff --git a/omni3d_amd/kernels/bnpool.py b/omni3d_amd/kernels/bnpool.py
--- a/omni3d_amd/kernels/bnpool.py
+++ b/omni3d_amd/kernels/bnpool.py
@@ -126,7 +126,7 @@
     coef = torch.empty(3 * C, dtype=torch.float32, device=x.device)
     ws = None
     if partials is not None:
-        assert partials.is_contiguous() and partials.shape[1] == 2 * C and res_carry is None and not dy_pitched
+        assert partials.is_contiguous() and partials.shape[1] == 2 * C and not dy_pitched
     else:
         ws = torch.empty(2 * C * 258, dtype=torch.float64, device=x.device)
     if res_carry is not None or dy_pitched:
@@ -166,6 +166,23 @@
     L.call("omni_maxpool2_bwd_carry", _lib.ptr(xv), dy.data_ptr(), dy.stride(3), _lib.ptr(carry), carry.stride(3) if carry is not None else 0,
            _lib.ptr(dx), N, H, W, C, _lib.stream_of(x))
     return dx.permute(0, 3, 1, 2)
+
+
+def maxpool2_bwd_bn_bwd(x, dy, carry, bn_x, mean_rstd, relu):
+    from .conv import STATS_ROWS, _nblk_cell, _stats_buf
+    xv = _nhwc(x)
+    N, H, W, C = xv.shape
+    bv = bn_x.permute(0, 2, 3, 1)
+    assert (carry is None or tuple(carry.shape) == tuple(x.shape)) and tuple(dy.shape) == (N, C, H // 2, W // 2) and dy.stride(1) == 1
+    assert bv.is_contiguous() and tuple(bv.shape) == (N, H, W, C) and mean_rstd.numel() == 2 * C
+    L = _lib.check_device(xv, bv, mean_rstd)
+    dx = torch.empty((N, H, W, C), dtype=torch.float32, device=x.device)
+    stats = _stats_buf(C, x.device)
+    cell, addr = _nblk_cell()
+    L.call("omni_maxpool2_bwd_bn_bwd_stats", _lib.ptr(xv), dy.data_ptr(), dy.stride(3), _lib.ptr(carry),
+           carry.stride(3) if carry is not None else 0, _lib.ptr(dx), N, H, W, C, _lib.ptr(bv), _lib.ptr(mean_rstd), int(bool(relu)),
+           _lib.ptr(stats), STATS_ROWS, addr, _lib.stream_of(x))
+    return dx.permute(0, 3, 1, 2), (stats[:cell.value] if cell.value > 0 else None)
 
 
 def avgpool2_fwd(x):
diff --git a/omni3d_amd/kernels/conv.py b/omni3d_amd/kernels/conv.py
--- a/omni3d_amd/kernels/conv.py
+++ b/omni3d_amd/kernels/conv.py
@@ -336,6 +336,24 @@
     return dx.permute(0, 3, 1, 2)
 
 
+def stem_conv_dgrad_bn_bwd(dy, w, in_hw, stride, bn_x, mean_rstd, scale_shift, bn_y=None):
+    dyv, wv = _nhwc(dy), _nhwc(w)
+    N, OH, OW, K = dyv.shape
+    H, W = in_hw
+    xv = bn_x.permute(0, 2, 3, 1)
+    assert (OH, OW) == ((H - 1) // stride + 1, (W - 1) // stride + 1) and tuple(wv.shape) == (K, 3, 3, 16)
+    assert xv.is_contiguous() and tuple(xv.shape) == (N, H, W, 16) and mean_rstd.numel() == 32
+    yv = bn_y.permute(0, 2, 3, 1) if bn_y is not None else None
+    assert yv is None or (yv.is_contiguous() and tuple(yv.shape) == (N, H, W, 16))
+    L = _lib.check_device(dyv, wv, xv, mean_rstd, scale_shift, yv)
+    dx = torch.empty((N, H, W, 16), dtype=torch.float32, device=dy.device)
+    stats = _stats_buf(16, dy.device)
+    cell, addr = _nblk_cell()
+    L.call("omni_stem_conv_dgrad_bn_bwd_stats", _lib.ptr(dyv), _lib.ptr(wv), _lib.ptr(dx), N, H, W, 16, K, 3, stride, K, 16, _lib.ptr(xv),
+           _lib.ptr(mean_rstd), _lib.ptr(scale_shift), _lib.ptr(yv), _lib.ptr(stats), STATS_ROWS, addr, _lib.stream_of(dy))
+    return dx.permute(0, 3, 1, 2), (stats[:cell.value] if cell.value > 0 else None)
+
+
 _STEM_WGRAD_ALL = os.environ.get("OMNI_STEM_WGRAD_ALL", "1") != "0"
 
 
diff --git a/omni3d_amd/kernels/wino.py b/omni3d_amd/kernels/wino.py
--- a/omni3d_amd/kernels/wino.py
+++ b/omni3d_amd/kernels/wino.py
@@ -334,7 +334,7 @@
     elif bn_below is not None and tile == 4:
         dx, parts = transform_output_bn_bwd(gemm_batched(Vd, U_flip), (N, H, W), *bn_below[:3])
         if parts is not None:
-            dx._omni_bn_bwd_parts = (parts, bn_below[1])
+            dx._omni_bn_bwd_parts = (parts, bn_below[1], dx._version)
     else:
         dx = transform_output(gemm_batched(Vd, U_flip), (N, H, W))
     if side_run is None or accum_into is None:
```

Result: no change. 379.8 images/s, median of 4 (+0.0%).
